# IITD-COMPUTER-VISION-GROUP/Egomotion_with_Local_Loop_Closures

Hardware: AMD Instinct MI355X
Metric: GN iterations/sec (640x480 semi-dense) (higher is better)
Workload: dtype f32; 1 GPU; C2 (configs[2]: batch of 32 loop-closure candidate alignments): 32 different keyframes (own depth map each) against ONE current frame per batch, the reference's loop-closure shape, 640x480, 4-level pyramid, FCA Gauss-Newton, schedule [4, 7, 9, 12] (early exit off), per-call mask compaction included, arithmetic mode 'fast' (pose <= 1e-5 vs the CPU path, tests/test_gpu_fast.py), 16 batches in flight; batch_per_gpu=32, global_batch=32, batches_in_flight=16, coalesce=4, launcher=single process, pixels=semi-dense (maxAbsGradient>=5), arith=fast, cpu_affinity=none

## Files before the change

egomotion_with_local_loop_closures_amd/_lib.py:

```python
import ctypes as C
import os
import subprocess

_HERE = os.path.dirname(os.path.abspath(__file__))
CSRC = os.path.join(_HERE, "csrc")
SO_PATH = os.path.join(CSRC, "libellc_hip.so")
MAX_LEVELS = 8

ABI_SYMBOLS = [
    "ellc_abi_version", "ellc_device_count", "ellc_default_config", "ellc_ctx_create", "ellc_ctx_destroy", "ellc_last_error", "ellc_sync", "ellc_stream", "ellc_ctx_counters", "ellc_ctx_set_poll_timeout_us", "ellc_ctx_set_grid_batch", "ellc_ctx_set_dense_maps", "ellc_ctx_set_persistent_schedule",
    "ellc_frame_upload", "ellc_keyframe_upload", "ellc_keyframe_from_frame", "ellc_get_image_level", "ellc_get_gradient",
    "ellc_get_max_gradient", "ellc_keyframe_set_depth", "ellc_keyframe_set_depth_level", "ellc_keyframe_get_depth_level",
    "ellc_keyframe_set_weights", "ellc_keyframe_get_weights", "ellc_keyframe_finalise_weights", "ellc_align", "ellc_align_enqueue",
    "ellc_align_fetch", "ellc_align_quality_at", "ellc_gn_iterate", "ellc_gn_display_planes", "ellc_concatenate_relative_pose", "ellc_concatenate_origin_pose", "ellc_se3_exp",
    "ellc_se3_log", "ellc_depth_set_state", "ellc_depth_get_state", "ellc_depth_set_keyframe", "ellc_depth_propagate",
    "ellc_depth_observe", "ellc_depth_fill_holes", "ellc_depth_regularize", "ellc_depth_make_inv_depth_one", "ellc_depth_regularize_fill_regularize", "ellc_depth_do_regularization",
    "ellc_depth_update_depth_image", "ellc_depth_create_keyframe", "ellc_depth_seeds", "ellc_track_frame",
    "ellc_histogram", "ellc_kl_divergence", "ellc_copy_slot", "ellc_copy_slot_across",
    "ellc_ingest_configure", "ellc_frame_ingest_bgr",
    "ellc_shard_range", "ellc_comm_unique_id", "ellc_comm_init_rccl", "ellc_comm_init_tcp", "ellc_comm_info", "ellc_comm_destroy", "ellc_comm_last_error",
    "ellc_gather_start", "ellc_gather_finish", "ellc_gather_results",
]


DIAG_SYMBOLS = [
    "ellc_profile_gn_kernel", "ellc_profile_align", "ellc_profile_depth_stage", "ellc_profile_calibrate_read", "ellc_profile_stream_read",
    "ellc_selftest_div_pair", "ellc_selftest_lu", "ellc_debug_persist_delay", "ellc_debug_set_persist_epoch", "ellc_debug_persist_counters", "ellc_debug_set_eager_lists", "ellc_debug_set_hinv_cache", "ellc_debug_set_fold_staging",
    "ellc_debug_set_count_cache", "ellc_debug_count_cache_counters",
    "ellc_debug_schedule_sums",
]


class EllcConfig(C.Structure):
    _fields_ = [("width", C.c_int), ("height", C.c_int), ("levels", C.c_int),
                ("fx", C.c_float), ("fy", C.c_float), ("cx", C.c_float), ("cy", C.c_float),
                ("max_iter", C.c_int * MAX_LEVELS), ("early_exit", C.c_int),
                ("max_keyframes", C.c_int), ("max_frames", C.c_int), ("max_batch", C.c_int), ("device", C.c_int),
                ("concurrent_batches", C.c_int), ("arith", C.c_int), ("coalesce", C.c_int), ("cache_records", C.c_int), ("grid_batch", C.c_int)]


class EllcHypotheses(C.Structure):
    _fields_ = [("invDepth", C.c_void_p), ("invDepthSmoothed", C.c_void_p), ("variance", C.c_void_p), ("varianceSmoothed", C.c_void_p),
                ("validity_counter", C.c_void_p), ("blacklisted", C.c_void_p), ("isValid", C.c_void_p)]


class EllcAlignQuality(C.Structure):
    _fields_ = [("n_depth", C.c_int32), ("n_used", C.c_int32),
                ("sum_r2", C.c_double), ("sum_abs_r", C.c_double), ("sum_w", C.c_double), ("sum_wr2", C.c_double),
                ("H", C.c_float * 36), ("b", C.c_float * 6), ("Hinv", C.c_float * 36)]


class EllcError(RuntimeError):
    pass


def build(verbose=False):
    args = ["make", "-C", CSRC]
    if not verbose:
        args.insert(1, "-s")
    subprocess.check_call(args)

# ... 67 lines not shown
```

egomotion_with_local_loop_closures_amd/api.py:

```python
import ctypes as C
import numpy as np
from . import _lib
from ._lib import EllcConfig, EllcHypotheses, EllcAlignQuality, EllcError, MAX_LEVELS

MODE_FCA = 0
MODE_ICA = 1
ARITH_EXACT = 0
ARITH_FAST = 1
HYP_FIELDS = ("invDepth", "invDepthSmoothed", "variance", "varianceSmoothed", "validity", "blacklisted", "valid")


def _p(a):
    return None if a is None else a.ctypes.data_as(C.c_void_p)


def default_config(width, height, levels=4, **kw):
    cfg = EllcConfig()
    _lib.lib().ellc_default_config(C.byref(cfg), width, height, levels)
    for k, v in kw.items():
        if k == "max_iter":
            mi = list(v) + [12] * (MAX_LEVELS - len(v))
            for i in range(MAX_LEVELS):
                cfg.max_iter[i] = mi[i]
        else:
# ... 271 lines not shown
        self._ck(self._l.ellc_histogram(self.h, int(is_kf), slot, _p(h)), "ellc_histogram")
        return h

    def copy_slot(self, dst_is_kf, dst, src_is_kf, src):
        self._ck(self._l.ellc_copy_slot(self.h, int(dst_is_kf), dst, int(src_is_kf), src), "ellc_copy_slot")

    def _need_diag(self, what):
        if not self.diag and _lib.DIAG_SO_PATH != _lib.SO_PATH:
            raise EllcError("%s is a diagnostic entry point (include/ellc_abi_diag.h): create the context with diag=True" % what)

    def debug_persist_delay(self, first_block, polls):
        self._need_diag("ellc_debug_persist_delay")
        self._ck(self._l.ellc_debug_persist_delay(self.h, int(first_block), int(polls)), "ellc_debug_persist_delay")

    def debug_set_persist_epoch(self, epoch):
        self._need_diag("ellc_debug_set_persist_epoch")
        self._ck(self._l.ellc_debug_set_persist_epoch(self.h, C.c_uint(epoch)), "ellc_debug_set_persist_epoch")

    def debug_set_eager_lists(self, on):
        self._need_diag("ellc_debug_set_eager_lists")
        self._ck(self._l.ellc_debug_set_eager_lists(self.h, int(bool(on))), "ellc_debug_set_eager_lists")

    def debug_set_fold_staging(self, on):
        self._need_diag("ellc_debug_set_fold_staging")
        self._ck(self._l.ellc_debug_set_fold_staging(self.h, int(bool(on))), "ellc_debug_set_fold_staging")

    def debug_set_hinv_cache(self, on):
        self._need_diag("ellc_debug_set_hinv_cache")
        self._ck(self._l.ellc_debug_set_hinv_cache(self.h, int(bool(on))), "ellc_debug_set_hinv_cache")

    def debug_set_count_cache(self, on):
        self._need_diag("ellc_debug_set_count_cache")
        self._ck(self._l.ellc_debug_set_count_cache(self.h, int(bool(on))), "ellc_debug_set_count_cache")

    def debug_count_cache_counters(self):
        self._need_diag("ellc_debug_count_cache_counters")
        a = C.c_longlong(0); b = C.c_longlong(0)
        self._ck(self._l.ellc_debug_count_cache_counters(self.h, C.byref(a), C.byref(b)), "ellc_debug_count_cache_counters")
        return a.value, b.value

    def debug_persist_counters(self):
        self._need_diag("ellc_debug_persist_counters")
        a = C.c_longlong(0); b = C.c_longlong(0); r = C.c_longlong(0)
        self._ck(self._l.ellc_debug_persist_counters(self.h, C.byref(a), C.byref(b), C.byref(r)), "ellc_debug_persist_counters")
        return a.value, b.value, r.value

    def debug_schedule_sums(self, kf_slots, frame_slots, level, pose, mode=MODE_FCA):
        self._need_diag("ellc_debug_schedule_sums")
        B = len(kf_slots)
        pose = np.ascontiguousarray(np.broadcast_to(np.asarray(pose, np.float32).reshape(-1, 6), (B, 6)), np.float32)
        _, kf, fr, _ = self._batch(kf_slots, frame_slots, None)
        sums = np.zeros((B, 27), np.float64); newp = np.zeros((B, 6), np.float32); hinv = np.zeros((B, 36), np.float32)
        name = C.create_string_buffer(64); grid = np.zeros(3, np.int32)
        self._ck(self._l.ellc_debug_schedule_sums(self.h, B, _p(kf), _p(fr), level, mode, _p(pose), _p(sums), _p(newp), _p(hinv), name, 64,
                                                  _p(grid)), "ellc_debug_schedule_sums")
        H = np.zeros((B, 6, 6), np.float64)
        iu = np.triu_indices(6)
        H[:, iu[0], iu[1]] = sums[:, :21]
        H[:, iu[1], iu[0]] = sums[:, :21]
        return dict(H=H, b=sums[:, 21:].copy(), pose=newp, hinv=hinv.reshape(B, 6, 6), kernel=name.value.decode(),
                    grid=tuple(int(v) for v in grid))

    def profile_gn_kernel(self, kf_slots, frame_slots, level, reps=20):
        self._need_diag("ellc_profile_gn_kernel")
        B, kf, fr, _ = self._batch(kf_slots, frame_slots, None)
        ms = C.c_float(0); by = C.c_double(0); v = C.c_longlong(0)
# ... 85 lines not shown
```

egomotion_with_local_loop_closures_amd/csrc/ellc_context.hpp:

```cpp
#pragma once
#include <hip/hip_runtime.h>
#include <string>
#include <vector>
#include <array>
#include <map>
#include <tuple>
#include "../../include/ellc_abi.h"
#ifdef ELLC_DIAG_ABI
#include "../../include/ellc_abi_diag.h"
#endif
#include "ellc_device.hpp"

namespace ellc {

struct DepthSoA {
  float* invDepth = nullptr;
  float* invDepthSmoothed = nullptr;
  float* variance = nullptr;
  float* varianceSmoothed = nullptr;
  int* validity = nullptr;
  int* blacklisted = nullptr;
  uint8_t* isValid = nullptr;
};

struct LaunchPlan {
  int B = 0;
  int nu = 0;
  int mode = ELLC_MODE_FCA;
  int save_weights = 0;
  int set = 0;
  bool continuation = false;
  bool dense = false;
  int need = 0;
  bool skip_count = false;
  bool pollable = false;
  bool resident = false;
  int adaptive_first = 0;
  bool direct = false;
  bool track = false;
  const void* count_valid = nullptr;
  int count_n = 0;
};

struct TrackRequest {
  const void* count_valid;
  int count_n;
};

struct GraphKey {
  int B, nu, mode, save_weights, continuation, track, pollable, adaptive_first, grid_batch, dense, need, skip_count, set;
  bool operator<(const GraphKey& o) const {
    auto t = [](const GraphKey& k) {
      return std::tie(k.B, k.nu, k.mode, k.save_weights, k.continuation, k.track, k.pollable, k.adaptive_first, k.grid_batch, k.dense, k.need, k.skip_count, k.set);
    };
    return t(*this) < t(o);
  }
};
inline GraphKey graph_key(const LaunchPlan& p, int grid_batch) {
  return GraphKey{p.B, p.nu, p.mode, p.save_weights ? 1 : 0, p.continuation, p.track, p.pollable, p.adaptive_first, grid_batch, p.dense, p.need, p.skip_count, p.set};
}

}

struct ellc_ctx {
  ellc_config cfg;
  hipStream_t stream = nullptr;
  std::string err;
  int L = 0;
  ellc::LevelGeom geom_h[ELLC_MAX_LEVELS];
  ellc::LevelGeom* geom_d = nullptr;
  std::vector<void*> allocs;
  char* arena_base = nullptr;
  size_t arena_size = 0, arena_used = 0;
  bool fast = false;
  std::vector<void*> host_allocs;
  std::vector<ellc::KfLevelDev> kf_tab_h;
  std::vector<ellc::FrLevelDev> fr_tab_h;
  ellc::KfLevelDev* kf_tab_d = nullptr;
  ellc::FrLevelDev* fr_tab_d = nullptr;
  std::vector<char> kf_has_image, kf_has_depth, fr_has_image;
  std::vector<char> kf_dense;
  bool dense_maps_off = false;
#ifdef ELLC_NO_DENSE_QUADS
  bool dense_quads = false;
#else
  bool dense_quads = true;
#endif
  std::vector<int> kf_rec_tag;
  std::vector<char> kf_rec_eager;
  bool eager_lists = true;
  bool fold_staging = true;
  std::vector<char> kf_hinv_ok;
  bool hinv_cache = true;
  std::vector<char> kf_counts_ok;
  bool count_cache = true;
  long long groups_counted = 0, groups_count_skipped = 0;
  bool cache_records = false;
  std::vector<std::array<int, ELLC_MAX_LEVELS>> kf_num_weights;
  std::vector<float*> kf_maxgrad, fr_maxgrad;
  std::vector<int*> kf_maxgrad_count, fr_maxgrad_count;
  std::vector<char> kf_maxgrad_valid, fr_maxgrad_valid;
  int *kf_slot_d = nullptr, *fr_slot_d = nullptr, *uniq_slot_d = nullptr;
  int *kf_slot_h = nullptr, *fr_slot_h = nullptr, *uniq_slot_h = nullptr;
  float *init_pose_d = nullptr, *init_pose_h = nullptr;
  ellc::AlignState *state_d = nullptr, *state_h = nullptr;
  ellc::AlignResult* result_h = nullptr;
  ellc::AlignResult* result_dev_alias = nullptr;
// ... 118 lines not shown
  int track_counts = 0;
  int* track_dev_alias = nullptr;
  float Kinv[9], Kmat[9];
};

namespace ellc {
ellc_status fail(ellc_ctx* c, ellc_status s, const std::string& msg);
ellc_status enqueue_eager_lists(ellc_ctx* c, int slot);
void invalidate_records(ellc_ctx* c, int slot);
void invalidate_lists(ellc_ctx* c, int slot);
#define ELLC_HIP(ctx, expr)                                                                               \
  do {                                                                                                    \
    hipError_t e__ = (expr);                                                                              \
    if (e__ != hipSuccess) return ellc::fail(ctx, ELLC_ERR_HIP, std::string(#expr) + ": " + hipGetErrorString(e__)); \
  } while (0)

ellc_status enter(ellc_ctx* c, bool join);
#define ELLC_ENTER_IMPL(ctx, join)                      \
  do {                                                  \
    if (ctx) {                                          \
      const ellc_status s__ = ellc::enter(ctx, join);   \
      if (s__ != ELLC_OK) return s__;                   \
    }                                                   \
  } while (0)
#define ELLC_ENTER(ctx) ELLC_ENTER_IMPL(ctx, true)
#define ELLC_ENTER_BATCH(ctx) ELLC_ENTER_IMPL(ctx, false)

int choose_nblk(const ellc_ctx* c, int level, int B, bool dense);
ellc_status run_prep(ellc_ctx* c, const LaunchPlan& p);
ellc_status build_depth_pyramid(ellc_ctx* c, int slot);
ellc_status build_depth_pyramid_from(ellc_ctx* c, int slot, int first_level);
ellc_status build_maxgrad(ellc_ctx* c, bool is_kf, int slot);
ellc_status build_image_pyramid(ellc_ctx* c, uint8_t* const* img, hipStream_t st);
ellc_status mark_frame_use(ellc_ctx* c, int slot);
}
```

egomotion_with_local_loop_closures_amd/csrc/ellc_device.hpp:

```cpp
#pragma once
#include <hip/hip_runtime.h>
#include <stdint.h>

#define ELLC_MAX_LEVELS 8
#define ELLC_PART_STRIDE 32
#define ELLC_NBLK_MAX 256
#define ELLC_GN_THREADS 256

namespace ellc {

struct LevelGeom {
  int cols, rows, sw, sh;
  int n;
  float fx, fy, cx, cy;
  float rfx, rfy;
  int divc_ok;
  const double* colA;
  const float* colB;
  const double* rowA;
  const float* rowB;
};

struct __attribute__((packed, aligned(4))) FcaRec {
  uint32_t xyI;
// ... 5 lines not shown
  uint32_t xyI;
  float var, d;
};

struct __attribute__((aligned(16))) IcaRec {
  float X, Y, Z, Ikf;
  float W, sd0, sd1, sd2;
  float sd3, sd4, sd5, pad;
};

struct KfLevelDev {
  uint8_t* img;
  float* depth;
  float* var;
  float* weight;
  uint32_t* cxy;
  float* cZ;
  float* cI;
  FcaRec* crec;
  IcaRec* irec;
  float* hpart;
  float* hinv;
  float* cW;
  float* wlast;
  float* sd;
  int* count;
  int* tile_count;
  float* idepth;
  double* invz;
};

struct FrLevelDev {
  uint8_t* img;
};

#define DM_OBS_REGIONS 64

struct AlignState {
  float pose[6];
  float S[12];
  float delta[6];
  float weighted;
  int level_done;
  int pending;
  int cur_level;
  int it_in_level;
  int iters[ELLC_MAX_LEVELS];
  float H[36];
  float b[6];
  float Hinv[36];
};

struct AlignResult {
  float pose[6];
  float weighted;
  int iters[ELLC_MAX_LEVELS];
  int pad;
};

}
```

egomotion_with_local_loop_closures_amd/csrc/ellc_hip.hip:

```cpp
#include "ellc_context.hpp"
#include "ellc_kernels_image.hpp"
#include "ellc_kernels_gn.hpp"
#include "ellc_kernels_prep.hpp"
#include <cstring>
#include <cmath>
#include <algorithm>
#include <cstdlib>
#include <map>
#include <chrono>
#include <thread>
#include <atomic>
#include <mutex>

using namespace ellc;

static ellc_status resolve_batch(ellc_ctx* c, int set);
static ellc_status launch_group(ellc_ctx* c, int set);

namespace ellc {

ellc_status fail(ellc_ctx* c, ellc_status s, const std::string& msg) {
  if (c) c->err = msg;
  return s;
}
// ... 88 lines not shown
  const bool share = c->cfg.concurrent_batches > 1 && (double)n / (256.0 * per_full) < 100.0;
  const int per = std::max(1, per_full / (share ? 2 : 1));
  int nblk = std::min(ELLC_NBLK_MAX, std::min(by_px, per));
  const int cus = std::max(1, c->resident_blocks / blocks_per_cu);
  if (nblk * B > cus) {
    const int one_per_cu = std::max(1, cus / B);
    if (0.3 * n / (256.0 * one_per_cu) <= 4.0) nblk = std::min(nblk, one_per_cu);
  }
  if (B <= 2 && c->use_fused && c->use_adaptive && c->cfg.early_exit && c->cfg.grid_batch == 0) nblk = std::min(nblk, 128);
  return nblk;
}

static dim3 grid2d(int w, int h, dim3 blk) { return dim3((w + blk.x - 1) / blk.x, (h + blk.y - 1) / blk.y); }

ellc_status build_image_pyramid(ellc_ctx* c, uint8_t* const* img, hipStream_t st) {
  const LevelGeom* g = c->geom_h;
  for (int l = 0; l + 1 < c->L; l += 3) {
    PyrChainArgs a;
    a.steps = std::min(3, c->L - 1 - l);
    a.src = img[l];
    for (int k = 0; k < 4; k++) {
      const int q = std::min(l + k, c->L - 1);
      a.w[k] = g[q].sw;
      a.h[k] = g[q].sh;
    }
    for (int k = 0; k < 3; k++) a.dst[k] = img[std::min(l + 1 + k, c->L - 1)];
    const int dw = g[l + a.steps].sw, dh = g[l + a.steps].sh;
    hipLaunchKernelGGL(pyr_down_chain_u8, dim3((dw + ELLC_PT - 1) / ELLC_PT, (dh + ELLC_PT - 1) / ELLC_PT), dim3(256), 0, st, a);
  }
  ELLC_HIP(c, hipGetLastError());
  return ELLC_OK;
}

static ellc_status upload_pyramid(ellc_ctx* c, uint8_t* const* img, const uint8_t* host, int frame_slot = -1) {
  const LevelGeom* g = c->geom_h;
  hipStream_t st = c->stream;
  if (frame_slot >= 0) {
    if (!c->upload_stream) {
      ELLC_HIP(c, hipStreamCreateWithFlags(&c->upload_stream, hipStreamNonBlocking));
      c->fr_use_ev.assign(c->cfg.max_frames, nullptr);
      c->fr_ready_ev.assign(c->cfg.max_frames, nullptr);
      hipEvent_t all = nullptr;
      ELLC_HIP(c, hipEventCreateWithFlags(&all, hipEventDisableTiming));
      hipError_t e = hipEventRecord(all, c->stream);
      if (e == hipSuccess) e = hipStreamWaitEvent(c->upload_stream, all, 0);
      (void)hipEventDestroy(all);
      ELLC_HIP(c, e);
    }
    st = c->upload_stream;
    if (c->fr_use_ev[frame_slot]) ELLC_HIP(c, hipStreamWaitEvent(st, c->fr_use_ev[frame_slot], 0));
    for (int p = 0; p < ellc_ctx::SETS; p++)
      if (c->batch_set[p].launched) ELLC_HIP(c, hipStreamWaitEvent(st, c->batch_set[p].done, 0));
  }
  const size_t bytes = (size_t)g[0].sw * g[0].sh;
  const int k = c->upload_cursor;
  c->upload_cursor = (c->upload_cursor + 1) % ellc_ctx::UPLOAD_RING;
  if (!c->upload_stage[k]) {
    ELLC_HIP(c, hipHostMalloc((void**)&c->upload_stage[k], bytes, hipHostMallocDefault));
    ELLC_HIP(c, hipEventCreateWithFlags(&c->upload_done[k], hipEventDisableTiming));
  } else {
    ELLC_HIP(c, hipEventSynchronize(c->upload_done[k]));
  }
  std::memcpy(c->upload_stage[k], host, bytes);
  {
    void* stage_dev = nullptr;
    ELLC_HIP(c, hipHostGetDevicePointer(&stage_dev, c->upload_stage[k], 0));
    const int blocks = (int)std::min<size_t>(1024, ((bytes >> 4) + 255) / 256 + 1);
    hipLaunchKernelGGL(ingest_copy_u8, dim3(blocks), dim3(256), 0, st, img[0], (const uint8_t*)stage_dev, bytes);
  }
  const ellc_status s = build_image_pyramid(c, img, st);
  ELLC_HIP(c, hipEventRecord(c->upload_done[k], st));
  if (s != ELLC_OK || frame_slot < 0) return s;
  if (!c->fr_ready_ev[frame_slot]) ELLC_HIP(c, hipEventCreateWithFlags(&c->fr_ready_ev[frame_slot], hipEventDisableTiming));
  ELLC_HIP(c, hipEventRecord(c->fr_ready_ev[frame_slot], st));
  ELLC_HIP(c, hipStreamWaitEvent(c->stream, c->fr_ready_ev[frame_slot], 0));
  return ELLC_OK;
}

ellc_status mark_frame_use(ellc_ctx* c, int slot) {
  if (!c->upload_stream) return ELLC_OK;
  if (!c->fr_use_ev[slot]) ELLC_HIP(c, hipEventCreateWithFlags(&c->fr_use_ev[slot], hipEventDisableTiming));
  ELLC_HIP(c, hipEventRecord(c->fr_use_ev[slot], c->stream));
  return ELLC_OK;
}

ellc_status build_maxgrad(ellc_ctx* c, bool is_kf, int slot) {
  const LevelGeom& g = c->geom_h[0];
  const uint8_t* img = is_kf ? c->kf_tab_h[slot].img : c->fr_tab_h[slot].img;
  float* out = is_kf ? c->kf_maxgrad[slot] : c->fr_maxgrad[slot];
  int* cnt = is_kf ? c->kf_maxgrad_count[slot] : c->fr_maxgrad_count[slot];
  ELLC_HIP(c, hipMemsetAsync(cnt, 0, sizeof(int), c->stream));
  hipLaunchKernelGGL(maxgrad_fused, dim3((g.cols + 31) / 32, (g.rows + 7) / 8), dim3(256), 0, c->stream, img, g.sw, g.cols, g.rows, out, cnt);
  ELLC_HIP(c, hipGetLastError());
  (is_kf ? c->kf_maxgrad_valid : c->fr_maxgrad_valid)[slot] = 1;
  return ELLC_OK;
}

ellc_status build_depth_pyramid(ellc_ctx* c, int slot) { return build_depth_pyramid_from(c, slot, 1); }

ellc_status build_depth_pyramid_from(ellc_ctx* c, int slot, int first_level) {
  for (int l = std::max(1, first_level); l < c->L; l++) {
    const KfLevelDev& s = c->kf_tab_h[(l - 1) * c->cfg.max_keyframes + slot];
    const KfLevelDev& d = c->kf_tab_h[l * c->cfg.max_keyframes + slot];
// ... 48 lines not shown
  ELLC_HIP(c, hipGetLastError());
  return ELLC_OK;
}

ellc_status run_prep(ellc_ctx* c, const LaunchPlan& p) { return run_prep_levels(c, p, 0, c->L - 1, c->stream); }

static void enqueue_ica_hinv(ellc_ctx* c, int n_unique) {
  const PrepArgs a = prep_args(c, 4, 0);
  hipLaunchKernelGGL(ica_hinv, dim3(c->L, n_unique), dim3(ELLC_SOLVE_THREADS), 0, c->stream, a);
}

static bool slot_ok(int s, int n) { return s >= 0 && s < n; }

static int grid_batch(const ellc_ctx* c, int B) {
  if (c->cfg.grid_batch > 0) return c->cfg.grid_batch;
  return (c->coalesce > 1 && B % c->cfg.max_batch == 0) ? c->cfg.max_batch * c->coalesce : B;
}

static GnArgs make_gn_args(ellc_ctx* c, const LaunchPlan& p, int level, int save_w, float* planes) {
  GnArgs a;
  a.geom = c->geom_d;
  a.kf_tab = c->kf_tab_d;
  a.fr_tab = c->fr_tab_d;
  a.kf_slot = c->kf_slot_d;
  a.fr_slot = c->fr_slot_d;
  a.state = c->state_d;
  a.partials = c->partials_d;
  a.planes = planes;
  a.level = level;
  a.max_kf = c->cfg.max_keyframes;
  a.max_fr = c->cfg.max_frames;
  a.nblk = choose_nblk(c, level, grid_batch(c, p.B), p.dense);
  a.save_w = save_w;
  return a;
}

static void launch_fca(ellc_ctx* c, dim3 grd, dim3 blk, const GnArgs& a) {
  if (c->fast) hipLaunchKernelGGL((gn_fca_accumulate<false, false, true>), grd, blk, 0, c->stream, a);
  else if (c->geom_h[0].divc_ok) hipLaunchKernelGGL((gn_fca_accumulate<false, true>), grd, blk, 0, c->stream, a);
  else hipLaunchKernelGGL((gn_fca_accumulate<false, false>), grd, blk, 0, c->stream, a);
}

#if defined(__x86_64__)
__attribute__((target("fma")))
#endif
static bool verify_div_const_fma(float b) {
  const float rb = (float)(1.0 / (double)b);
  for (uint32_t m = 0; m < (1u << 23); m++) {
    uint32_t bits = 0x3f800000u | m;
    float a;
    std::memcpy(&a, &bits, 4);
    const float q = a * rb;
    const float e = __builtin_fmaf(-b, q, a);
    const float r = __builtin_fmaf(e, rb, q);
    if (r != a / b) return false;
  }
  return true;
}
static bool verify_div_const(float b) {
  static std::map<uint32_t, bool> cache;
  static std::mutex cache_mutex;
  std::lock_guard<std::mutex> lock(cache_mutex);
  if (!(b > 0.0f) || !std::isfinite(b)) return false;
#if defined(__x86_64__)
  if (!__builtin_cpu_supports("fma")) return false;
#elif !defined(__FP_FAST_FMAF)
// ... 504 lines not shown
        copy_blocking(c, dRB, rowB.data(), g.rows * 4, hipMemcpyHostToDevice) != hipSuccess) {
      *out = c;
      return fail(c, ELLC_ERR_HIP, "cannot upload the Jacobian tables");
    }
    g.colA = dA; g.rowA = dR; g.colB = dB; g.rowB = dRB;
    c->cap[l] = g.n;
    c->tile_begin[l + 1] = c->tile_begin[l] + (g.n + ELLC_TILE - 1) / ELLC_TILE;
    sw = (sw + 1) / 2;
    sh = (sh + 1) / 2;
  }
  TRY(dev_alloc(c, &c->geom_d, ELLC_MAX_LEVELS));
  if (copy_blocking(c, c->geom_d, c->geom_h, sizeof(LevelGeom) * c->L, hipMemcpyHostToDevice) != hipSuccess) {
    *out = c;
    return fail(c, ELLC_ERR_HIP, "cannot upload the level geometry");
  }
  const int MK = cfg->max_keyframes, MF = cfg->max_frames;
  c->kf_tab_h.assign((size_t)c->L * MK, KfLevelDev());
  c->fr_tab_h.assign((size_t)c->L * MF, FrLevelDev());
  for (int l = 0; l < c->L; l++) {
    const LevelGeom& g = c->geom_h[l];
    const size_t n = g.n, ni = (size_t)g.sw * g.sh;
    const int tiles = c->tile_begin[l + 1] - c->tile_begin[l];
    for (int s = 0; s < MK; s++) {
      KfLevelDev& k = c->kf_tab_h[(size_t)l * MK + s];
      TRY(dev_alloc(c, &k.img, ni + 16));
      TRY(dev_alloc(c, &k.depth, n)); TRY(dev_alloc(c, &k.var, n)); TRY(dev_alloc(c, &k.weight, n));
      TRY(dev_alloc(c, &k.cxy, n)); TRY(dev_alloc(c, &k.cZ, n)); TRY(dev_alloc(c, &k.cI, n));
      TRY(dev_alloc(c, &k.crec, n)); TRY(dev_alloc(c, &k.cW, n)); TRY(dev_alloc(c, &k.wlast, n)); TRY(dev_alloc(c, &k.sd, 6 * n));
      TRY(dev_alloc(c, &k.count, 4)); TRY(dev_alloc(c, &k.tile_count, tiles + 1)); TRY(dev_alloc(c, &k.idepth, n));
      k.invz = nullptr;
      if (!c->fast) TRY(dev_alloc(c, &k.invz, n));
      TRY(dev_alloc(c, &k.irec, n)); TRY(dev_alloc(c, &k.hpart, (size_t)(tiles + 1) * ELLC_PART_STRIDE)); TRY(dev_alloc(c, &k.hinv, 36));
    }
    for (int s = 0; s < MF; s++) TRY(dev_alloc(c, &c->fr_tab_h[(size_t)l * MF + s].img, ni + (size_t)g.sw + 32));
  }
  TRY(dev_alloc(c, &c->kf_tab_d, c->kf_tab_h.size()));
  TRY(dev_alloc(c, &c->fr_tab_d, c->fr_tab_h.size()));
  if (copy_blocking(c, c->kf_tab_d, c->kf_tab_h.data(), c->kf_tab_h.size() * sizeof(KfLevelDev), hipMemcpyHostToDevice) != hipSuccess ||
      copy_blocking(c, c->fr_tab_d, c->fr_tab_h.data(), c->fr_tab_h.size() * sizeof(FrLevelDev), hipMemcpyHostToDevice) != hipSuccess) {
    *out = c;
    return fail(c, ELLC_ERR_HIP, "cannot upload the slot tables");
  }
  c->kf_has_image.assign(MK, 0); c->kf_has_depth.assign(MK, 0); c->fr_has_image.assign(MF, 0);
  c->kf_dense.assign(MK, 0);
  c->kf_num_weights.assign(MK, std::array<int, ELLC_MAX_LEVELS>{});
  c->kf_rec_tag.assign(MK, 0);
  c->kf_rec_eager.assign(MK, 0);
  c->kf_hinv_ok.assign(MK, 0);
  c->kf_counts_ok.assign(MK, 0);
  c->cache_records = cfg->cache_records != 0;
  c->kf_maxgrad.assign(MK, nullptr); c->fr_maxgrad.assign(MF, nullptr);
  c->kf_maxgrad_count.assign(MK, nullptr); c->fr_maxgrad_count.assign(MF, nullptr);
  c->kf_maxgrad_valid.assign(MK, 0); c->fr_maxgrad_valid.assign(MF, 0);
  const size_t n0 = (size_t)cfg->width * cfg->height;
  for (int s = 0; s < MK; s++) { TRY(dev_alloc(c, &c->kf_maxgrad[s], n0)); TRY(dev_alloc(c, &c->kf_maxgrad_count[s], 4)); }
  for (int s = 0; s < MF; s++) { TRY(dev_alloc(c, &c->fr_maxgrad[s], n0)); TRY(dev_alloc(c, &c->fr_maxgrad_count[s], 4)); }
  const int MB = cfg->max_batch;
  c->coalesce = std::max(1, cfg->coalesce);
  c->group_cap = c->coalesce * MB;
  c->max_inflight = c->coalesce > 1 ? (ellc_ctx::STREAMS + 1) * c->coalesce : ellc_ctx::STREAMS;
  c->n_sets = c->max_inflight + 1;
  c->batch_stream[0] = c->stream;
  const size_t CAP = (size_t)c->group_cap;
  for (int p = 0; p < c->n_sets; p++) {
    ellc_ctx::BatchSet& bs = c->batch_set[p];
    TRY(dev_alloc(c, &bs.stage_d, 9 * CAP));
    TRY(host_alloc(c, &bs.stage_h, 9 * CAP));
// ... 182 lines not shown
}
ellc_status ellc_debug_set_persist_epoch(ellc_ctx* c, unsigned epoch) {
  if (!c) return ELLC_ERR_BAD_ARG;
  ELLC_ENTER(c);
  c->persist_epoch = epoch;
  return ELLC_OK;
}
ellc_status ellc_debug_set_eager_lists(ellc_ctx* c, int on) {
  if (!c) return ELLC_ERR_BAD_ARG;
  ELLC_ENTER(c);
  c->eager_lists = on != 0;
  if (!on) std::fill(c->kf_rec_eager.begin(), c->kf_rec_eager.end(), 0);
  return ELLC_OK;
}
ellc_status ellc_debug_set_fold_staging(ellc_ctx* c, int on) {
  if (!c) return ELLC_ERR_BAD_ARG;
  ELLC_ENTER(c);
  c->fold_staging = on != 0;
  c->ride_saved_weights = on != 0;
  return ELLC_OK;
}
ellc_status ellc_debug_set_hinv_cache(ellc_ctx* c, int on) {
  if (!c) return ELLC_ERR_BAD_ARG;
  ELLC_ENTER(c);
  c->hinv_cache = on != 0;
  return ELLC_OK;
}
ellc_status ellc_debug_set_count_cache(ellc_ctx* c, int on) {
  if (!c) return ELLC_ERR_BAD_ARG;
  ELLC_ENTER(c);
  c->count_cache = on != 0;
  return ELLC_OK;
}
ellc_status ellc_debug_count_cache_counters(ellc_ctx* c, long long* groups_counted, long long* groups_skipped) {
  if (!c) return ELLC_ERR_BAD_ARG;
  ELLC_ENTER(c);
  if (groups_counted) *groups_counted = c->groups_counted;
  if (groups_skipped) *groups_skipped = c->groups_count_skipped;
  return ELLC_OK;
}
ellc_status ellc_debug_persist_counters(ellc_ctx* c, long long* resident_launches, long long* abandoned_launches, long long* rejoined_blocks) {
  if (!c) return ELLC_ERR_BAD_ARG;
  ELLC_ENTER(c);
  if (resident_launches) *resident_launches = c->persist_launches;
  if (abandoned_launches) *abandoned_launches = c->persist_abandoned;
  if (rejoined_blocks) {
    unsigned long long v = 0;
    ELLC_HIP(c, hipDeviceSynchronize());
    ELLC_HIP(c, hipMemcpyFromSymbol(&v, HIP_SYMBOL(ellc::g_persist_adoptions), sizeof(v)));
    *rejoined_blocks = (long long)v;
  }
  return ELLC_OK;
}
#endif

ellc_status ellc_ctx_set_dense_maps(ellc_ctx* c, int mode) {
  ELLC_ENTER_BATCH(c);
  if (!c || mode < 0 || mode > 1) return fail(c, ELLC_ERR_BAD_ARG, "ellc_ctx_set_dense_maps: mode 0 (automatic) or 1 (always the lists)");
  if (c->open_set >= 0) {
    const ellc_status s = launch_group(c, c->open_set);
    if (s != ELLC_OK) return s;
  }
  c->dense_maps_off = mode == 1;
  return ELLC_OK;
}

ellc_status ellc_ctx_set_grid_batch(ellc_ctx* c, int n) {
  ELLC_ENTER_BATCH(c);
  if (!c || n < 0 || n > 65536) return fail(c, ELLC_ERR_BAD_ARG, "bad argument");
  if (c->open_set >= 0) {
    const ellc_status s = launch_group(c, c->open_set);
    if (s != ELLC_OK) return s;
  }
  c->cfg.grid_batch = n;
  return ELLC_OK;
}

ellc_status ellc_frame_upload(ellc_ctx* c, int slot, const uint8_t* image) {
  ELLC_ENTER(c);
  if (!c || !image || !slot_ok(slot, c->cfg.max_frames)) return fail(c, ELLC_ERR_BAD_ARG, "ellc_frame_upload: bad argument");
  uint8_t* img[ELLC_MAX_LEVELS];
  for (int l = 0; l < c->L; l++) img[l] = c->fr_tab_h[(size_t)l * c->cfg.max_frames + slot].img;
  const bool own_stream = c->cfg.concurrent_batches <= 1 && c->coalesce <= 1;
  ellc_status s = upload_pyramid(c, img, image, own_stream ? slot : -1);
  if (s != ELLC_OK) return s;
  c->fr_has_image[slot] = 1;
  c->fr_maxgrad_valid[slot] = 0;
  return ELLC_OK;
}

ellc_status ellc_keyframe_upload(ellc_ctx* c, int slot, const uint8_t* image) {
  ELLC_ENTER(c);
  if (!c || !image || !slot_ok(slot, c->cfg.max_keyframes)) return fail(c, ELLC_ERR_BAD_ARG, "ellc_keyframe_upload: bad argument");
  uint8_t* img[ELLC_MAX_LEVELS];
  for (int l = 0; l < c->L; l++) img[l] = c->kf_tab_h[(size_t)l * c->cfg.max_keyframes + slot].img;
  invalidate_records(c, slot);
  ellc_status s = upload_pyramid(c, img, image);
  if (s != ELLC_OK) return s;
  c->kf_has_image[slot] = 1;
  c->kf_dense[slot] = 0;
  c->kf_has_depth[slot] = 0;
  for (int l = 0; l < c->L; l++) {
    ELLC_HIP(c, hipMemsetAsync(c->kf_tab_h[(size_t)l * c->cfg.max_keyframes + slot].weight, 0, (size_t)c->geom_h[l].n * 4, c->stream));
    c->kf_num_weights[slot][l] = 0;
  }
  return build_maxgrad(c, true, slot);
}

ellc_status ellc_keyframe_from_frame(ellc_ctx* c, int kf_slot, int frame_slot) {
  ELLC_ENTER(c);
  if (!c || !slot_ok(kf_slot, c->cfg.max_keyframes) || !slot_ok(frame_slot, c->cfg.max_frames)) return fail(c, ELLC_ERR_BAD_ARG, "bad slot");
  if (!c->fr_has_image[frame_slot]) return fail(c, ELLC_ERR_NOT_READY, "frame slot empty");
  invalidate_records(c, kf_slot);
  for (int l = 0; l < c->L; l++) {
    const LevelGeom& g = c->geom_h[l];
    ELLC_HIP(c, hipMemcpyAsync(c->kf_tab_h[(size_t)l * c->cfg.max_keyframes + kf_slot].img, c->fr_tab_h[(size_t)l * c->cfg.max_frames + frame_slot].img,
                               (size_t)g.sw * g.sh, hipMemcpyDeviceToDevice, c->stream));
// ... 187 lines not shown
      KfLevelDev& d = dc->kf_tab_h[(size_t)l * MK + dst];
      if (src_is_kf) {
        const KfLevelDev& k = sc->kf_tab_h[(size_t)l * SK + src];
        ELLC_HIP(c, hipMemcpyAsync(d.depth, k.depth, (size_t)g.n * 4, hipMemcpyDeviceToDevice, dc->stream));
        ELLC_HIP(c, hipMemcpyAsync(d.var, k.var, (size_t)g.n * 4, hipMemcpyDeviceToDevice, dc->stream));
        if (sc->kf_dense[src]) ELLC_HIP(c, hipMemcpyAsync(d.idepth, k.idepth, (size_t)g.n * 4, hipMemcpyDeviceToDevice, dc->stream));
        if (sc->kf_dense[src] && d.invz) {
          if (k.invz) ELLC_HIP(c, hipMemcpyAsync(d.invz, k.invz, (size_t)g.n * 8, hipMemcpyDeviceToDevice, dc->stream));
          else hipLaunchKernelGGL(invz_plane, dim3((g.n + 255) / 256), dim3(256), 0, dc->stream, d.depth, d.invz, g.n);
        }
        ELLC_HIP(c, hipMemcpyAsync(d.weight, k.weight, (size_t)g.n * 4, hipMemcpyDeviceToDevice, dc->stream));
        dc->kf_num_weights[dst][l] = sc->kf_num_weights[src][l];
      } else {
        ELLC_HIP(c, hipMemsetAsync(d.weight, 0, (size_t)g.n * 4, dc->stream));
        dc->kf_num_weights[dst][l] = 0;
      }
    }
  }
  if (dst_is_kf) {
    dc->kf_has_image[dst] = 1;
    dc->kf_has_depth[dst] = src_is_kf ? sc->kf_has_depth[src] : 0;
    dc->kf_dense[dst] = src_is_kf ? sc->kf_dense[src] : 0;
    if (src_is_kf && sc->kf_maxgrad_valid[src]) {
      const size_t n0 = (size_t)dc->cfg.width * dc->cfg.height;
      ELLC_HIP(c, hipMemcpyAsync(dc->kf_maxgrad[dst], sc->kf_maxgrad[src], n0 * 4, hipMemcpyDeviceToDevice, dc->stream));
      ELLC_HIP(c, hipMemcpyAsync(dc->kf_maxgrad_count[dst], sc->kf_maxgrad_count[src], 4, hipMemcpyDeviceToDevice, dc->stream));
      dc->kf_maxgrad_valid[dst] = 1;
    } else {
      return build_maxgrad(dc, true, dst);
    }
  } else {
    dc->fr_has_image[dst] = 1;
    dc->fr_maxgrad_valid[dst] = 0;
  }
  return ELLC_OK;
}
static ellc_status mark_copy_uses(ellc_ctx* dc, int dst_is_kf, int dst, ellc_ctx* sc, int src_is_kf, int src) {
  ellc_status s = ELLC_OK;
  if (!src_is_kf) s = mark_frame_use(sc, src);
  if (s == ELLC_OK && !dst_is_kf && dc == sc) s = mark_frame_use(dc, dst);
  return s;
}

ellc_status ellc_copy_slot(ellc_ctx* c, int dst_is_kf, int dst, int src_is_kf, int src) {
  ELLC_ENTER(c);
  if (!c || !slot_ok(dst, dst_is_kf ? c->cfg.max_keyframes : c->cfg.max_frames) || !slot_ok(src, src_is_kf ? c->cfg.max_keyframes : c->cfg.max_frames))
    return fail(c, ELLC_ERR_BAD_ARG, "bad slot");
  if (!(src_is_kf ? c->kf_has_image[src] : c->fr_has_image[src])) return fail(c, ELLC_ERR_NOT_READY, "source slot empty");
  if (dst_is_kf == src_is_kf && dst == src) return ELLC_OK;
  const ellc_status st = copy_slot_planes(c, dst_is_kf, dst, c, src_is_kf, src);
  return st != ELLC_OK ? st : mark_copy_uses(c, dst_is_kf, dst, c, src_is_kf, src);
}

ellc_status ellc_copy_slot_across(ellc_ctx* dc, int dst_is_kf, int dst, ellc_ctx* sc, int src_is_kf, int src) {
  if (!dc || !sc) return ELLC_ERR_BAD_ARG;
  if (dc == sc) return ellc_copy_slot(dc, dst_is_kf, dst, src_is_kf, src);
  if (dc->cfg.device != sc->cfg.device || dc->cfg.width != sc->cfg.width || dc->cfg.height != sc->cfg.height || dc->L != sc->L)
    return fail(dc, ELLC_ERR_BAD_ARG, "ellc_copy_slot_across: the contexts differ in device or geometry");
  if (!slot_ok(dst, dst_is_kf ? dc->cfg.max_keyframes : dc->cfg.max_frames) || !slot_ok(src, src_is_kf ? sc->cfg.max_keyframes : sc->cfg.max_frames))
    return fail(dc, ELLC_ERR_BAD_ARG, "bad slot");
  if (!(src_is_kf ? sc->kf_has_image[src] : sc->fr_has_image[src])) return fail(dc, ELLC_ERR_NOT_READY, "source slot empty");
  {
    ellc_ctx* c = sc;
    ELLC_ENTER(c);
    if (!sc->ev_xfer) ELLC_HIP(c, hipEventCreateWithFlags(&sc->ev_xfer, hipEventDisableTiming));
    ELLC_HIP(c, hipEventRecord(sc->ev_xfer, sc->stream));
// ... 4 lines not shown
  ELLC_HIP(c, hipStreamWaitEvent(dc->stream, sc->ev_xfer, 0));
  const ellc_status st = copy_slot_planes(dc, dst_is_kf, dst, sc, src_is_kf, src);
  ELLC_HIP(c, hipEventRecord(dc->ev_xfer, dc->stream));
  if (hipStreamWaitEvent(sc->stream, dc->ev_xfer, 0) != hipSuccess) return fail(sc, ELLC_ERR_HIP, "ellc_copy_slot_across: cannot order the source stream");
  sc->main_dirty = true;
  return st;
}

static int need_of(const ellc_ctx* c, int mode) {
  return mode == ELLC_MODE_ICA ? (c->use_fused ? (c->fast ? 20 : 4) : 1) : (c->fast ? 8 : 2);
}

static bool runs_dense(const ellc_ctx* c, int mode, int B, int save_weights) {
  return !c->dense_maps_off && c->use_fused && c->pipe && mode == ELLC_MODE_FCA && !save_weights && !schedule_is_adaptive(c, mode, B);
}
static bool group_is_dense(const ellc_ctx* c, int mode, int B, int save_weights, const int* slots, int n) {
  bool dense = runs_dense(c, mode, B, save_weights);
  for (int i = 0; i < n; i++) dense = dense && c->kf_dense[slots[i]];
  return dense;
}

static LaunchPlan make_plan(const ellc_ctx* c, int B, int nu, int mode, int save_weights, int set, bool dense, bool resident) {
  LaunchPlan p;
  p.B = B;
  p.nu = dense ? 0 : nu;
  p.mode = mode;
  p.save_weights = save_weights;
  p.set = set;
  p.dense = dense;
  p.need = need_of(c, mode);
  p.resident = resident;
  p.adaptive_first = schedule_is_adaptive(c, mode, B) ? adaptive_first_launches(c, resident) : 0;
  p.direct = launches_directly(c, mode, B);
  return p;
}

static ellc_status enqueue_align_body(ellc_ctx* c, const LaunchPlan& p) {
  enqueue_stage_in(c, p, p.B);
  ellc_status s = ELLC_OK;
  if (p.nu > 0) {
    s = run_prep(c, p);
    if (s != ELLC_OK) return s;
    if (p.need & 4) enqueue_ica_hinv(c, p.nu);
  }
  s = enqueue_schedule(c, p);
  if (s != ELLC_OK) return s;
  if (!c->use_fused)
    hipLaunchKernelGGL(gn_export_results, dim3((p.B + 63) / 64), dim3(64), 0, c->stream, c->state_d, c->result_dev_alias, p.B);
  return ELLC_OK;
}

static ellc_status launch_align_graph(ellc_ctx* c, const LaunchPlan& p, bool count_twin = false) {
  auto body = [&](const LaunchPlan& q) -> ellc_status { return q.continuation ? enqueue_schedule_adaptive(c, q) : enqueue_align_body(c, q); };
  if (p.direct) return body(p);
  auto capture = [&](const LaunchPlan& q) -> ellc_status {
    hipGraph_t graph = nullptr;
    hipGraphExec_t exec = nullptr;
    ELLC_HIP(c, hipStreamBeginCapture(c->stream, hipStreamCaptureModeThreadLocal));
    const ellc_status s = body(q);
    hipError_t e = hipStreamEndCapture(c->stream, &graph);
    if (s != ELLC_OK || e != hipSuccess) {
      if (graph) (void)hipGraphDestroy(graph);
      if (s != ELLC_OK) return s;
      return fail(c, ELLC_ERR_HIP, std::string("hipStreamEndCapture: ") + hipGetErrorString(e));
    }
    e = hipGraphInstantiate(&exec, graph, nullptr, nullptr, 0);
// ... 331 lines not shown
  if (last) free_set(c, set);
  return out;
}

ellc_status ellc_align(ellc_ctx* c, int B, const int* kf_slots, const int* frame_slots, const float* init_pose, int mode, int save_weights,
                       float* out_pose, int* out_iters, float* out_weighted) {
  ELLC_ENTER(c);
  if (c && c->n_inflight > 0) return fail(c, ELLC_ERR_NOT_READY, "ellc_align: fetch the enqueued batches first");
  ellc_status s = ellc_align_enqueue(c, B, kf_slots, frame_slots, init_pose, mode, save_weights);
  if (s != ELLC_OK) return s;
  return ellc_align_fetch(c, B, out_pose, out_iters, out_weighted);
}

__global__ void gn_set_pose0(AlignState* state, const float* pose) {
  AlignState& st = state[0];
  float p[6], S[12];
  for (int i = 0; i < 6; i++) { p[i] = pose[i]; st.pose[i] = p[i]; }
  exp_se3_f32(p, S);
  for (int i = 0; i < 12; i++) st.S[i] = S[i];
  st.level_done = -1;
}

ellc_status ellc_gn_iterate(ellc_ctx* c, int kf_slot, int frame_slot, int level, int mode, int iter, const float* pose, float* H36, float* b6,
                            float* delta6, float* new_pose6, float* weighted, float* planes) {
  ELLC_ENTER(c);
  if (!c || !pose || level < 0 || level >= c->L) return fail(c, ELLC_ERR_BAD_ARG, "bad argument");
  if (c->n_inflight > 0) return fail(c, ELLC_ERR_NOT_READY, "ellc_gn_iterate: fetch the enqueued batches first");
  int nu = 0;
  select_batch_set(c, 0);
  invalidate_records(c, kf_slot);
  ellc_status s = stage_batch(c, 1, &kf_slot, &frame_slot, pose, &nu);
  if (s != ELLC_OK) return s;
  LaunchPlan plan;
  plan.B = 1;
  plan.nu = nu;
  plan.mode = mode;
  plan.need = mode == ELLC_MODE_ICA ? 1 : (c->fast ? 8 : 2);
  enqueue_stage_in(c, plan, 0);
  s = run_prep(c, plan);
  if (s != ELLC_OK) return s;
  hipLaunchKernelGGL(gn_set_pose0, dim3(1), dim3(1), 0, c->stream, c->state_d, c->init_pose_d);
  const size_t n = (size_t)c->geom_h[level].n;
  if (planes) ELLC_HIP(c, hipMemsetAsync(c->planes_d, 0, 10 * n * 4, c->stream));
  GnArgs a = make_gn_args(c, plan, level, 0, planes ? c->planes_d : nullptr);
  const dim3 grd(a.nblk, 1), blk(ELLC_GN_THREADS);
  if (mode == ELLC_MODE_FCA) {
    if (planes && c->fast) hipLaunchKernelGGL((gn_fca_accumulate<true, false, true>), grd, blk, 0, c->stream, a);
    else if (planes && c->geom_h[0].divc_ok) hipLaunchKernelGGL((gn_fca_accumulate<true, true>), grd, blk, 0, c->stream, a);
    else if (planes) hipLaunchKernelGGL((gn_fca_accumulate<true, false>), grd, blk, 0, c->stream, a);
    else launch_fca(c, grd, blk, a);
    launch_solve(c, level, 1, a.nblk, 0, 0);
  } else {
    if (iter == 0) {
      hipLaunchKernelGGL(gn_ica_precompute, grd, blk, 0, c->stream, a, c->cap[level]);
      launch_solve(c, level, 1, a.nblk, 1, 0);
    }
    if (planes) hipLaunchKernelGGL(gn_ica_iterate<true>, grd, blk, 0, c->stream, a, c->cap[level]);
    else hipLaunchKernelGGL(gn_ica_iterate<false>, grd, blk, 0, c->stream, a, c->cap[level]);
    launch_solve(c, level, 1, a.nblk, 2, 0);
  }
  ELLC_HIP(c, hipGetLastError());
  ELLC_HIP(c, hipMemcpyAsync(c->state_h, c->state_d, sizeof(AlignState), hipMemcpyDeviceToHost, c->stream));
  if (planes) {
    ELLC_HIP(c, hipMemcpyAsync(planes, c->planes_d, 10 * n * 4, hipMemcpyDeviceToHost, c->stream));
  }
  ELLC_HIP(c, hipStreamSynchronize(c->stream));
// ... 35 lines not shown
  if (!c->quality_out_h) {
    const size_t nb0 = (size_t)quality_nblk(c, 0);
    ellc_status s = host_alloc(c, &c->quality_stage_h, (size_t)8 * MB);
    if (s == ELLC_OK) s = dev_alloc(c, &c->quality_partials_d, (size_t)MB * nb0 * ELLC_PART_STRIDE);
    if (s == ELLC_OK) s = dev_alloc(c, &c->quality_counts_d, (size_t)MB * nb0 * 2);
    ellc_align_quality* oh = nullptr;
    if (s == ELLC_OK) s = host_alloc(c, &oh, (size_t)MB);
    if (s != ELLC_OK) return s;
    void *da = nullptr, *ds = nullptr;
    ELLC_HIP(c, hipHostGetDevicePointer(&da, oh, 0));
    ELLC_HIP(c, hipHostGetDevicePointer(&ds, c->quality_stage_h, 0));
    c->quality_out_dev_alias = (ellc_align_quality*)da;
    c->quality_stage_dev_alias = (const int*)ds;
    c->quality_out_h = oh;
  }
  for (int b = 0; b < B; b++) {
    c->quality_stage_h[b] = kf_slots[b];
    c->quality_stage_h[MB + b] = frame_slots[b];
  }
  std::memcpy(c->quality_stage_h + 2 * MB, pose, (size_t)B * 6 * sizeof(float));
  QualityArgs qa;
  qa.geom = c->geom_d;
  qa.kf_tab = c->kf_tab_d;
  qa.fr_tab = c->fr_tab_d;
  qa.stage = c->quality_stage_dev_alias;
  qa.partials = c->quality_partials_d;
  qa.counts = c->quality_counts_d;
  qa.out = (QualityRec*)c->quality_out_dev_alias;
  qa.level = level;
  qa.max_kf = c->cfg.max_keyframes;
  qa.max_fr = c->cfg.max_frames;
  qa.nblk = quality_nblk(c, level);
  qa.max_batch = MB;
  const dim3 grd(qa.nblk, B), blk(ELLC_GN_THREADS);
  if (c->fast) hipLaunchKernelGGL((gn_fca_quality<true, false>), grd, blk, 0, c->stream, qa);
  else if (c->geom_h[0].divc_ok) hipLaunchKernelGGL((gn_fca_quality<false, true>), grd, blk, 0, c->stream, qa);
  else hipLaunchKernelGGL((gn_fca_quality<false, false>), grd, blk, 0, c->stream, qa);
  hipLaunchKernelGGL(gn_quality_finish, dim3(B), dim3(ELLC_SOLVE_THREADS), 0, c->stream, qa);
  ELLC_HIP(c, hipGetLastError());
  ELLC_HIP(c, hipStreamSynchronize(c->stream));
  std::memcpy(out, c->quality_out_h, (size_t)B * sizeof(ellc_align_quality));
  return ELLC_OK;
}

ellc_status ellc_gn_display_planes(ellc_ctx* c, int kf_slot, int frame_slot, int level, const float* pose, uint8_t* templateimg,
                                   uint8_t* tobewarpedimg, float* warpedimg, float* origres) {
  ELLC_ENTER(c);
  if (!c || !pose || level < 0 || level >= c->L) return fail(c, ELLC_ERR_BAD_ARG, "bad argument");
  if (c->n_inflight > 0) return fail(c, ELLC_ERR_NOT_READY, "ellc_gn_display_planes: fetch the enqueued batches first");
  int nu = 0;
  select_batch_set(c, 0);
  ellc_status s = stage_batch(c, 1, &kf_slot, &frame_slot, pose, &nu);
  if (s != ELLC_OK) return s;
  LaunchPlan plan;
  plan.B = 1;
  enqueue_stage_in(c, plan, 0);
  hipLaunchKernelGGL(gn_set_pose0, dim3(1), dim3(1), 0, c->stream, c->state_d, c->init_pose_d);
  const LevelGeom& g = c->geom_h[level];
  const size_t n = (size_t)g.n;
  float* warped_d = c->planes_d;
  float* orig_d = c->planes_d + n;
  uint8_t* tmpl_d = (uint8_t*)(c->planes_d + 2 * n);
  uint8_t* tbw_d = tmpl_d + n;
  GnArgs a = make_gn_args(c, plan, level, 0, nullptr);
  dim3 blk(32, 8);
  hipLaunchKernelGGL(gn_display_planes, grid2d(g.cols, g.rows, blk), blk, 0, c->stream, a, tmpl_d, tbw_d, warped_d, orig_d);
  ELLC_HIP(c, hipGetLastError());
  if (templateimg) ELLC_HIP(c, hipMemcpyAsync(templateimg, tmpl_d, n, hipMemcpyDeviceToHost, c->stream));
  if (tobewarpedimg) ELLC_HIP(c, hipMemcpyAsync(tobewarpedimg, tbw_d, n, hipMemcpyDeviceToHost, c->stream));
  if (warpedimg) ELLC_HIP(c, hipMemcpyAsync(warpedimg, warped_d, n * 4, hipMemcpyDeviceToHost, c->stream));
  if (origres) ELLC_HIP(c, hipMemcpyAsync(origres, orig_d, n * 4, hipMemcpyDeviceToHost, c->stream));
  ELLC_HIP(c, hipStreamSynchronize(c->stream));
  return ELLC_OK;
}

void ellc_concatenate_relative_pose(const float* a, const float* b, float* dest) {
  float o[6];
  concat_relative_f32(a, b, o);
  std::memcpy(dest, o, sizeof(o));
}
void ellc_concatenate_origin_pose(const float* a, const float* b, float* dest) {
  float o[6];
  concat_origin_f32(a, b, o);
  std::memcpy(dest, o, sizeof(o));
}
void ellc_se3_exp(const float* pose6, float* T16) {
  float S[12];
  exp_se3_f32(pose6, S);
  std::memcpy(T16, S, sizeof(S));
  T16[12] = T16[13] = T16[14] = 0.0f;
  T16[15] = 1.0f;
}
void ellc_se3_log(const float* T16, float* pose6) {
  float S[12];
  std::memcpy(S, T16, sizeof(S));
  log_se3_f32(S, pose6);
}

#ifdef ELLC_DIAG_ABI
ellc_status ellc_profile_gn_kernel(ellc_ctx* c, int B, const int* kf_slots, const int* frame_slots, int level, int reps, float* avg_ms,
                                   double* algorithmic_bytes, long long* valid_pixels) {
  ELLC_ENTER(c);
  if (!c || level < 0 || level >= c->L || reps < 1) return fail(c, ELLC_ERR_BAD_ARG, "bad argument");
  if (c->n_inflight > 0) return fail(c, ELLC_ERR_NOT_READY, "ellc_profile_gn_kernel: fetch the enqueued batches first");
  int nu = 0;
  select_batch_set(c, 0);
  if (kf_slots)
    for (int b = 0; b < B; b++) invalidate_records(c, kf_slots[b]);
  ellc_status s = stage_batch(c, B, kf_slots, frame_slots, nullptr, &nu, nullptr, true);
  if (s != ELLC_OK) return s;
  const bool dense = group_is_dense(c, ELLC_MODE_FCA, B, 0, kf_slots, B);
  LaunchPlan plan;
  plan.B = B;
  plan.nu = dense ? 0 : nu;
  plan.dense = dense;
  plan.need = c->fast ? 8 : 2;
  enqueue_stage_in(c, plan, 0);
  if (!dense) {
    s = run_prep(c, plan);
    if (s != ELLC_OK) return s;
  }
  hipLaunchKernelGGL(gn_init_state, dim3((B + 63) / 64), dim3(64), 0, c->stream, c->state_d, c->init_pose_d, B, c->L - 1);
  const GnArgs a = make_gn_args(c, plan, level, 0, nullptr);
  const dim3 grd(a.nblk, B), blk(ELLC_GN_THREADS);
  if (c->use_fused) {
    FusedArgs fa = fused_args(c, plan, false, (B % 8 == 0) ? 1 : 0, false);
    level_bound_level(c, plan, fa, level);
    fa.res = nullptr;
    fa.prev_level = level;
    fa.prev_nblk = a.nblk;
    fa.early_exit = 0;
    auto launch = [&]() {
      launch_level_bound(c, plan, grd, blk, fa, c->stream);
      fa.seq++;
    };
    for (int i = 0; i < 3; i++) launch();
    if (c->use_graph) {
      hipGraph_t graph = nullptr;
      hipGraphExec_t exec = nullptr;
      ELLC_HIP(c, hipStreamBeginCapture(c->stream, hipStreamCaptureModeThreadLocal));
      for (int i = 0; i < reps; i++) launch();
      hipError_t e = hipStreamEndCapture(c->stream, &graph);
      if (e == hipSuccess) e = hipGraphInstantiate(&exec, graph, nullptr, nullptr, 0);
      if (graph) (void)hipGraphDestroy(graph);
      if (e != hipSuccess) return fail(c, ELLC_ERR_HIP, std::string("profile graph capture: ") + hipGetErrorString(e));
// ... 272 lines not shown
```

egomotion_with_local_loop_closures_amd/csrc/ellc_ingest_impl.hpp:

```cpp
#pragma once
#include "ellc_context.hpp"
#include <cmath>
#include <vector>

namespace ellc {

struct IngestMapEntry {
  short ix, iy;
  unsigned short frac;
  unsigned short pad;
};

static inline void ingest_inv3x3(const double* S, double* t) {
  const double d0 = S[0] * (S[4] * S[8] - S[5] * S[7]) - S[1] * (S[3] * S[8] - S[5] * S[6]) + S[2] * (S[3] * S[7] - S[4] * S[6]);
  if (d0 == 0.0) { for (int i = 0; i < 9; i++) t[i] = 0.0; return; }
  const double d = 1. / d0;
  t[0] = (S[4] * S[8] - S[5] * S[7]) * d;
  t[1] = (S[2] * S[7] - S[1] * S[8]) * d;
  t[2] = (S[1] * S[5] - S[2] * S[4]) * d;
  t[3] = (S[5] * S[6] - S[3] * S[8]) * d;
  t[4] = (S[0] * S[8] - S[2] * S[6]) * d;
  t[5] = (S[2] * S[3] - S[0] * S[5]) * d;
  t[6] = (S[3] * S[7] - S[4] * S[6]) * d;
  t[7] = (S[1] * S[6] - S[0] * S[7]) * d;
// ... 135 lines not shown
  if (ie != hipSuccess) {
    if (c->ingest_map) (void)hipFree(c->ingest_map);
    if (c->ingest_bgr) (void)hipFree(c->ingest_bgr);
    c->ingest_map = nullptr;
    c->ingest_bgr = nullptr;
    return fail(c, ELLC_ERR_HIP, std::string("ellc_ingest_configure: ") + hipGetErrorString(ie));
  }
  c->ingest_w = orig_w;
  c->ingest_h = orig_h;
  return ELLC_OK;
}

ellc_status ellc_frame_ingest_bgr(ellc_ctx* c, int slot, const uint8_t* bgr, uint8_t* gray_probe, uint8_t* undistorted_probe) {
  ELLC_ENTER(c);
  using namespace ellc;
  if (!c || !bgr || !slot_ok(slot, c->cfg.max_frames)) return fail(c, ELLC_ERR_BAD_ARG, "ellc_frame_ingest_bgr: bad argument");
  if (!c->ingest_map) return fail(c, ELLC_ERR_NOT_READY, "ellc_frame_ingest_bgr: call ellc_ingest_configure first");
  const int w = c->ingest_w, h = c->ingest_h, ow = c->cfg.width, oh = c->cfg.height;
  ELLC_HIP(c, hipMemcpyAsync(c->ingest_bgr, bgr, (size_t)w * h * 3, hipMemcpyHostToDevice, c->stream));
  uint8_t *gd = nullptr, *ud = nullptr;
  if (gray_probe) ELLC_HIP(c, hipMalloc(&gd, (size_t)ow * oh));
  if (undistorted_probe && hipMalloc(&ud, (size_t)ow * oh * 4) != hipSuccess) {
    if (gd) (void)hipFree(gd);
    return fail(c, ELLC_ERR_HIP, "ellc_frame_ingest_bgr: cannot allocate the probe buffer");
  }
  uint8_t* img[ELLC_MAX_LEVELS];
  for (int l = 0; l < c->L; l++) img[l] = c->fr_tab_h[(size_t)l * c->cfg.max_frames + slot].img;
  const LevelGeom* g = c->geom_h;
  dim3 blk(32, 8);
  hipLaunchKernelGGL(ingest_frame, grid2d(ow, oh, blk), blk, 0, c->stream, c->ingest_bgr, w, h, (const IngestMapEntry*)c->ingest_map, img[0], ow, oh,
                     g[0].sw, gd, ud);
  hipError_t e = hipGetLastError();
  if (e == hipSuccess && build_image_pyramid(c, img, c->stream) != ELLC_OK) e = hipErrorUnknown;
  if (e == hipSuccess && gd) e = hipMemcpyAsync(gray_probe, gd, (size_t)ow * oh, hipMemcpyDeviceToHost, c->stream);
  if (e == hipSuccess && ud) e = hipMemcpyAsync(undistorted_probe, ud, (size_t)ow * oh * 4, hipMemcpyDeviceToHost, c->stream);
  if (e == hipSuccess) e = hipStreamSynchronize(c->stream);
  if (gd) (void)hipFree(gd);
  if (ud) (void)hipFree(ud);
  if (e != hipSuccess) return fail(c, ELLC_ERR_HIP, std::string("ellc_frame_ingest_bgr: ") + hipGetErrorString(e));
  c->fr_has_image[slot] = 1;
  c->fr_maxgrad_valid[slot] = 0;
  return ELLC_OK;
}

}
```

egomotion_with_local_loop_closures_amd/csrc/ellc_kernels_gn.hpp:

```cpp
#pragma once
#include "ellc_device.hpp"
#include "ellc_se3.hpp"

namespace ellc {

#ifdef ELLC_STAMPS
__device__ unsigned long long g_stamps[64];
__device__ unsigned long long g_block_stamps[4 * 8192];
#define ELLC_BSTAMP(slot)                                                                                    \
  do {                                                                                                       \
    if (threadIdx.x == 0) {                                                                                  \
      unsigned long long t__;                                                                                \
      asm volatile("s_memrealtime %0\n\ts_waitcnt lgkmcnt(0)" : "=s"(t__)::"memory");                        \
      const unsigned bid__ = blockIdx.y * gridDim.x + blockIdx.x;                                            \
      if (bid__ < 8192) g_block_stamps[bid__ * 4 + slot] = t__;                                              \
    }                                                                                                        \
  } while (0)
#define ELLC_STAMP(id)                                                                                       \
  do {                                                                                                       \
    if (blockIdx.x == 0 && blockIdx.y == 0 && threadIdx.x == 0) {                                            \
      unsigned long long t__;                                                                                \
      asm volatile("s_memrealtime %0\n\ts_waitcnt lgkmcnt(0)" : "=s"(t__)::"memory");                            \
      g_stamps[id] = t__;                                                                                    \
    }                                                                                                        \
// ... 35 lines not shown
      g_seq_stamps[(off) + ((seq) & 31)] = t__;                                                              \
    }                                                                                                        \
  } while (0)
#else
#define ELLC_SEQSTAMP(off, seq) do { } while (0)
#endif

#define ELLC_GLOBAL __attribute__((address_space(1)))
typedef const ELLC_GLOBAL uint8_t* g_u8;
typedef const ELLC_GLOBAL float* g_f32;
typedef const ELLC_GLOBAL double* g_f64;
typedef const ELLC_GLOBAL uint32_t* g_u32;
template <class T>
__device__ __forceinline__ const ELLC_GLOBAL T* as_global(const T* p) { return (const ELLC_GLOBAL T*)p; }
template <class T>
__device__ __forceinline__ ELLC_GLOBAL T* as_global_rw(T* p) { return (ELLC_GLOBAL T*)p; }

template <int CTRL, int RMASK>
__device__ __forceinline__ float dpp_add(float v) {
  const int x = __builtin_amdgcn_update_dpp(0, __builtin_bit_cast(int, v), CTRL, RMASK, 0xf, false);
  return v + __builtin_bit_cast(float, x);
}
__device__ __forceinline__ float unzero_f(float v) {
  const float C = 0x1.b7cdfep-34f;
  return (v < 0.0f) ? ((v > -C) ? -C : v) : ((v < C) ? C : v);
}

__device__ __forceinline__ int clampi(int v, int lo, int hi) { return v < lo ? lo : (v > hi ? hi : v); }

typedef uint32_t u32_align1 __attribute__((aligned(1)));
__device__ __forceinline__ uint32_t load_u32_unaligned(g_u8 base, unsigned byte_off) {
  return *(const ELLC_GLOBAL u32_align1*)(base + byte_off);
}
template <int N>
__device__ __forceinline__ float byte_f32(uint32_t w) { return (float)((w >> (8 * N)) & 0xffu); }

#define ELLC_LDS __attribute__((address_space(3)))

struct Taps {
  float I;
  float gx, gy;
};

template <bool WANT_GRAD, bool FAST, bool LAT = false>
__device__ __forceinline__ Taps tap_general(g_u8 img, int sw, int cols, int rows, float x1, float y1) {
  Taps o;
  const float fx0 = floorf(x1), fy0 = floorf(y1);
  const float wx = x1 - fx0, wy = y1 - fy0;
  const float omx = 1.0f - wx, omy = 1.0f - wy;
  if (x1 != x1 || y1 != y1) {
    o.I = -1.0f; o.gx = 0.0f; o.gy = 0.0f;
    return o;
  }
  const float nC = (float)(cols - 1), nR = (float)(rows - 1);
  const bool xf_bad = (fx0 < 0.0f) || (fx0 > nC);
  const bool xc_bad = (x1 < 0.0f) || (x1 > nC);
  const bool yf_bad = (fy0 < 0.0f) || (fy0 > nR);
  const bool yc_bad = (y1 < 0.0f) || (y1 > nR);
  const bool v00 = !(xf_bad || yf_bad), v01 = !(xc_bad || yf_bad), v10 = !(xf_bad || yc_bad), v11 = !(xc_bad || yc_bad);
  if (!(v00 || v01 || v10 || v11)) {
    o.I = -1.0f; o.gx = 0.0f; o.gy = 0.0f;
    return o;
  }
  const int x0 = (int)fminf(fmaxf(fx0, -4.0f), nC + 4.0f);
  const int y0 = (int)fminf(fmaxf(fy0, -4.0f), nR + 4.0f);
  const int xb = clampi(x0, 0, cols - 1), xc = clampi(x0 + 1, 0, cols - 1);
// ... 54 lines not shown
    const int xa = clampi(x0 - 1, 0, cols - 1), xd = clampi(x0 + 2, 0, cols - 1);
    const int ya = clampi(y0 - 1, 0, rows - 1), yd = clampi(y0 + 2, 0, rows - 1);
    const unsigned ra = __umul24((unsigned)ya, (unsigned)sw), rd = __umul24((unsigned)yd, (unsigned)sw);
    const float Pba = (float)img[rb + (unsigned)xa], Pbd = (float)img[rb + (unsigned)xd];
    const float Pca = (float)img[rc + (unsigned)xa], Pcd = (float)img[rc + (unsigned)xd];
    const float Pab = (float)img[ra + (unsigned)xb], Pac = (float)img[ra + (unsigned)xc];
    const float Pdb = (float)img[rd + (unsigned)xb], Pdc = (float)img[rd + (unsigned)xc];
    const float sx0 = (x0 <= 0 || x0 >= cols - 1) ? 1.0f : 0.5f;
    const float sx1 = (x0 + 1 <= 0 || x0 + 1 >= cols - 1) ? 1.0f : 0.5f;
    const float sy0 = (y0 <= 0 || y0 >= rows - 1) ? 1.0f : 0.5f;
    const float sy1 = (y0 + 1 <= 0 || y0 + 1 >= rows - 1) ? 1.0f : 0.5f;
    float g00 = sx0 * (Pbc - Pba), g01 = sx1 * (Pbd - Pbb), g10 = sx0 * (Pcc - Pca), g11 = sx1 * (Pcd - Pcb);
    g00 = v00 ? g00 : 0.0f; g01 = v01 ? g01 : 0.0f; g10 = v10 ? g10 : 0.0f; g11 = v11 ? g11 : 0.0f;
    float top = (omx * g00) + (wx * g01);
    float btm = (omx * g10) + (wx * g11);
    o.gx = (omy * top) + (wy * btm);
    float h00 = sy0 * (Pcb - Pab), h01 = sy0 * (Pcc - Pac), h10 = sy1 * (Pdb - Pbb), h11 = sy1 * (Pdc - Pbc);
    h00 = v00 ? h00 : 0.0f; h01 = v01 ? h01 : 0.0f; h10 = v10 ? h10 : 0.0f; h11 = v11 ? h11 : 0.0f;
    top = (omx * h00) + (wx * h01);
    btm = (omx * h10) + (wx * h11);
    o.gy = (omy * top) + (wy * btm);
    if (FAST) { o.gx *= 2.0f; o.gy *= 2.0f; }
  } else {
    o.gx = 0.0f; o.gy = 0.0f;
  }
  return o;
}

struct NoPrefetch { __device__ __forceinline__ void operator()() const {} };
template <class F> struct LatPF { F f; __device__ __forceinline__ void operator()() const { f(); } };
template <class T> struct is_lat_pf { static constexpr bool value = false; };
template <class F> struct is_lat_pf<LatPF<F>> { static constexpr bool value = true; };
template <class F> __device__ __forceinline__ LatPF<F> lat_pf(F f) { return LatPF<F>{f}; }
template <bool WANT_GRAD, bool FAST = false, class AfterIssue = NoPrefetch>
__device__ __forceinline__ Taps tap_point(g_u8 img, int sw, int cols, int rows, float x1, float y1, AfterIssue after_issue = AfterIssue()) {
  Taps o;
  const float fx0 = floorf(x1), fy0 = floorf(y1);
  const float wx = x1 - fx0, wy = y1 - fy0;
  const float omx = 1.0f - wx, omy = 1.0f - wy;
  const bool interior = (__builtin_amdgcn_fmed3f(fx0, 1.0f, (float)(cols - 3)) == fx0) & (__builtin_amdgcn_fmed3f(fy0, 1.0f, (float)(rows - 3)) == fy0);
  if (__builtin_amdgcn_ballot_w64(!interior) == 0ull) {
    const int x0 = (int)fx0, y0 = (int)fy0;
    uint32_t wa = 0, wb, wc, wd = 0;
    const unsigned ob = __umul24((unsigned)y0, (unsigned)sw) + (unsigned)x0 - 1u, oc = ob + (unsigned)sw;
    wb = load_u32_unaligned(img, ob);
    wc = load_u32_unaligned(img, oc);
    if (WANT_GRAD) { wa = load_u32_unaligned(img, ob - (unsigned)sw); wd = load_u32_unaligned(img, oc + (unsigned)sw); }
    __builtin_amdgcn_sched_barrier(0);
    after_issue();
    __builtin_amdgcn_sched_barrier(0);
    const float Pbb = byte_f32<1>(wb), Pbc = byte_f32<2>(wb), Pcb = byte_f32<1>(wc), Pcc = byte_f32<2>(wc);
    if (FAST) {
      const float top = __builtin_fmaf(wx, Pbc - Pbb, Pbb);
      const float btm = __builtin_fmaf(wx, Pcc - Pcb, Pcb);
      o.I = __builtin_fmaf(wy, btm - top, top);
      if (WANT_GRAD) {
        const float Pba = byte_f32<0>(wb), Pbd = byte_f32<3>(wb), Pca = byte_f32<0>(wc), Pcd = byte_f32<3>(wc);
        const float Pab = byte_f32<1>(wa), Pac = byte_f32<2>(wa), Pdb = byte_f32<1>(wd), Pdc = byte_f32<2>(wd);
        const float g00 = Pbc - Pba, g01 = Pbd - Pbb, g10 = Pcc - Pca, g11 = Pcd - Pcb;
        float t2 = __builtin_fmaf(wx, g01 - g00, g00);
        float b2 = __builtin_fmaf(wx, g11 - g10, g10);
        o.gx = __builtin_fmaf(wy, b2 - t2, t2);
        const float h00 = Pcb - Pab, h01 = Pcc - Pac, h10 = Pdb - Pbb, h11 = Pdc - Pbc;
        t2 = __builtin_fmaf(wx, h01 - h00, h00);
        b2 = __builtin_fmaf(wx, h11 - h10, h10);
        o.gy = __builtin_fmaf(wy, b2 - t2, t2);
      } else {
        o.gx = 0.0f; o.gy = 0.0f;
      }
      return o;
    }
    {
      const float top = (omx * Pbb) + (wx * Pbc);
      const float btm = (omx * Pcb) + (wx * Pcc);
      o.I = (omy * top) + (wy * btm);
    }
    if (WANT_GRAD) {
      const float Pba = byte_f32<0>(wb), Pbd = byte_f32<3>(wb), Pca = byte_f32<0>(wc), Pcd = byte_f32<3>(wc);
      const float Pab = byte_f32<1>(wa), Pac = byte_f32<2>(wa), Pdb = byte_f32<1>(wd), Pdc = byte_f32<2>(wd);
      const float g00 = 0.5f * (Pbc - Pba), g01 = 0.5f * (Pbd - Pbb), g10 = 0.5f * (Pcc - Pca), g11 = 0.5f * (Pcd - Pcb);
      float top = (omx * g00) + (wx * g01);
      float btm = (omx * g10) + (wx * g11);
      o.gx = (omy * top) + (wy * btm);
      const float h00 = 0.5f * (Pcb - Pab), h01 = 0.5f * (Pcc - Pac), h10 = 0.5f * (Pdb - Pbb), h11 = 0.5f * (Pdc - Pbc);
      top = (omx * h00) + (wx * h01);
      btm = (omx * h10) + (wx * h11);
      o.gy = (omy * top) + (wy * btm);
    } else {
      o.gx = 0.0f; o.gy = 0.0f;
    }
    return o;
  }
  after_issue();
  return tap_general<WANT_GRAD, FAST, is_lat_pf<AfterIssue>::value>(img, sw, cols, rows, x1, y1);
}

struct TapRows { g_u8 ra, rb, rc, rd; };
__device__ __forceinline__ TapRows tap_rows(g_u8 img, int sw) {
  TapRows r;
  r.rb = img - 1;
  r.ra = r.rb - sw;
  r.rc = r.rb + sw;
  r.rd = r.rc + sw;
  return r;
}
template <int N>
__device__ __forceinline__ float cvt_ubyte(uint32_t w) {
  float f;
  if (N == 0) asm("v_cvt_f32_ubyte0 %0, %1" : "=v"(f) : "v"(w));
  else if (N == 1) asm("v_cvt_f32_ubyte1 %0, %1" : "=v"(f) : "v"(w));
  else if (N == 2) asm("v_cvt_f32_ubyte2 %0, %1" : "=v"(f) : "v"(w));
  else asm("v_cvt_f32_ubyte3 %0, %1" : "=v"(f) : "v"(w));
  return f;
}
__device__ __forceinline__ int cvt_floor_i32(float x) {
  int i;
  asm("v_cvt_flr_i32_f32 %0, %1" : "=v"(i) : "v"(x));
  return i;
}
struct TapReq {
  uint32_t wa, wb, wc, wd;
  bool interior;
};
template <bool WANT_GRAD, class AfterIssue = NoPrefetch>
__device__ __forceinline__ TapReq tap_request_f(const TapRows& tr, int sw, int cols, int rows, float x1, float y1, AfterIssue after_issue = AfterIssue()) {
  TapReq q;
  q.wa = 0; q.wd = 0;
  const int x0 = cvt_floor_i32(x1), y0 = cvt_floor_i32(y1);
  const bool interior = ((unsigned)(x0 - 1) <= (unsigned)(cols - 4)) & ((unsigned)(y0 - 1) <= (unsigned)(rows - 4));
  q.interior = (__builtin_amdgcn_ballot_w64(!interior) == 0ull);
  q.wb = 0; q.wc = 0;
  if (q.interior) {
    const unsigned off = __umul24((unsigned)y0, (unsigned)sw) + (unsigned)x0;
#ifdef ELLC_X_LDSTAPS
    __shared__ uint32_t xl[4 * 1024 + 4];
    const unsigned o = (off >> 2) & 1023u, shb = (off & 3u) * 8u;
    q.wb = __builtin_amdgcn_alignbit(xl[o + 1], xl[o], shb);
    q.wc = __builtin_amdgcn_alignbit(xl[1024 + o + 1], xl[1024 + o], shb);
    if (WANT_GRAD) { q.wa = __builtin_amdgcn_alignbit(xl[2048 + o + 1], xl[2048 + o], shb); q.wd = __builtin_amdgcn_alignbit(xl[3072 + o + 1], xl[3072 + o], shb); }
#else
    q.wb = load_u32_unaligned(tr.rb, off);
    q.wc = load_u32_unaligned(tr.rc, off);
    if (WANT_GRAD) { q.wa = load_u32_unaligned(tr.ra, off); q.wd = load_u32_unaligned(tr.rd, off); }
#endif
    __builtin_amdgcn_sched_barrier(0);
    after_issue();
    __builtin_amdgcn_sched_barrier(0);
  } else {
    after_issue();
  }
  return q;
}
template <bool WANT_GRAD, bool LAT = false>
__device__ __forceinline__ Taps tap_finish_f(const TapReq& q, g_u8 img, int sw, int cols, int rows, float x1, float y1) {
  if (q.interior) {
    Taps o;
    const float wx = __builtin_amdgcn_fractf(x1), wy = __builtin_amdgcn_fractf(y1);
    const float Pbb = cvt_ubyte<1>(q.wb), Pbc = cvt_ubyte<2>(q.wb), Pcb = cvt_ubyte<1>(q.wc), Pcc = cvt_ubyte<2>(q.wc);
    const float top = __builtin_fmaf(wx, Pbc - Pbb, Pbb);
    const float btm = __builtin_fmaf(wx, Pcc - Pcb, Pcb);
    o.I = __builtin_fmaf(wy, btm - top, top);
    if (WANT_GRAD) {
      const float Pba = cvt_ubyte<0>(q.wb), Pbd = cvt_ubyte<3>(q.wb), Pca = cvt_ubyte<0>(q.wc), Pcd = cvt_ubyte<3>(q.wc);
      const float Pab = cvt_ubyte<1>(q.wa), Pac = cvt_ubyte<2>(q.wa), Pdb = cvt_ubyte<1>(q.wd), Pdc = cvt_ubyte<2>(q.wd);
      const float g00 = Pbc - Pba, g01 = Pbd - Pbb, g10 = Pcc - Pca, g11 = Pcd - Pcb;
      float t2 = __builtin_fmaf(wx, g01 - g00, g00);
      float b2 = __builtin_fmaf(wx, g11 - g10, g10);
      o.gx = __builtin_fmaf(wy, b2 - t2, t2);
      const float h00 = Pcb - Pab, h01 = Pcc - Pac, h10 = Pdb - Pbb, h11 = Pdc - Pbc;
      t2 = __builtin_fmaf(wx, h01 - h00, h00);
      b2 = __builtin_fmaf(wx, h11 - h10, h10);
      o.gy = __builtin_fmaf(wy, b2 - t2, t2);
    } else {
      o.gx = 0.0f; o.gy = 0.0f;
    }
    return o;
  }
  return tap_general<WANT_GRAD, true, LAT>(img, sw, cols, rows, x1, y1);
}

__device__ __forceinline__ float div_const(float a, float b, float rb) {
  const float q = a * rb;
  const float e = __builtin_fmaf(-b, q, a);
  return __builtin_fmaf(e, rb, q);
}

__device__ __forceinline__ void div_pair_ieee(float a0, float b0, float a1, float b1, float& q0, float& q1) {
  typedef float v2 __attribute__((ext_vector_type(2)));
  bool vd0, vd1, vn0, vn1;
  const v2 ds = {__builtin_amdgcn_div_scalef(a0, b0, false, &vd0), __builtin_amdgcn_div_scalef(a1, b1, false, &vd1)};
  const v2 ns = {__builtin_amdgcn_div_scalef(a0, b0, true, &vn0), __builtin_amdgcn_div_scalef(a1, b1, true, &vn1)};
  const v2 r = {__builtin_amdgcn_rcpf(ds.x), __builtin_amdgcn_rcpf(ds.y)};
  const v2 nds = -ds;
  const v2 f0 = __builtin_elementwise_fma(nds, r, (v2)(1.0f));
  const v2 f1 = __builtin_elementwise_fma(f0, r, r);
  const v2 mul = ns * f1;
  const v2 f2 = __builtin_elementwise_fma(nds, mul, ns);
// ... 46 lines not shown
  J[0] = jt0 + jb0;
  J[1] = jt1 + jb1;
  J[2] = jt2 + jb2;
  J[3] = jt3 + 0.0f;
  J[4] = 0.0f + jb4;
  J[5] = jt5 + jb5;
}

__device__ __forceinline__ float fca_weight(const Warp& w, float d, float residual, float gradx, float grady, float s,
                                            const LevelGeom& g, float tx, float ty, float tz) {
  const float gx = g.fx * gradx;
  const float gy = g.fy * grady;
  const float den = (w.pz * w.pz) * d;
  float g0, g1;
  div_pair_ieee(tx * w.pz - tz * w.px, den, ty * w.pz - tz * w.py, den, g0, g1);
  const float drpdd = gx * g0 + gy * g1;
  const float w_p = 1.0f / (16.0f + (s * drpdd) * drpdd);
  const float weighted_rp = fabsf(residual * sqrtf(w_p));
  const float wh = fabsf(weighted_rp < 1.5f ? 1.0f : 1.5f / weighted_rp);
  return wh * w_p;
}

struct GnArgs {
  const LevelGeom* geom;
  const KfLevelDev* kf_tab;
  const FrLevelDev* fr_tab;
  const int* kf_slot;
  const int* fr_slot;
  AlignState* state;
  float* partials;
  float* planes;
  int level, max_kf, max_fr, nblk;
  int save_w;
};

template <int NV>
struct WaveRows {
  static constexpr int N1 = (NV + 1) / 2, N2 = (N1 + 1) / 2;
};
template <int NV>
__device__ __forceinline__ void wave_sum_rows(const float (&v)[NV], float (&out)[WaveRows<NV>::N2]) {
  constexpr int N1 = WaveRows<NV>::N1, N2 = WaveRows<NV>::N2;
  float s1[N1];
#pragma unroll
  for (int j = 0; j < N1; j++) {
    const float a = v[2 * j], b = (2 * j + 1 < NV) ? v[2 * j + 1] : 0.0f;
    const auto t = __builtin_amdgcn_permlane32_swap(__builtin_bit_cast(unsigned, a), __builtin_bit_cast(unsigned, b), false, false);
    const unsigned t0 = t[0], t1 = t[1];
    s1[j] = __builtin_bit_cast(float, t0) + __builtin_bit_cast(float, t1);
  }
#pragma unroll
  for (int j = 0; j < N2; j++) {
    const float a = s1[2 * j], b = (2 * j + 1 < N1) ? s1[2 * j + 1] : 0.0f;
    const auto t = __builtin_amdgcn_permlane16_swap(__builtin_bit_cast(unsigned, a), __builtin_bit_cast(unsigned, b), false, false);
    const unsigned t0 = t[0], t1 = t[1];
    out[j] = __builtin_bit_cast(float, t0) + __builtin_bit_cast(float, t1);
  }
#pragma unroll
  for (int j = 0; j < N2; j++) out[j] = dpp_add<0xB1, 0xf>(out[j]);
#pragma unroll
  for (int j = 0; j < N2; j++) out[j] = dpp_add<0x4E, 0xf>(out[j]);
#pragma unroll
  for (int j = 0; j < N2; j++) out[j] = dpp_add<0x141, 0xf>(out[j]);
#pragma unroll
  for (int j = 0; j < N2; j++) out[j] = dpp_add<0x140, 0xf>(out[j]);
}

// ... 98 lines not shown
  const Warp w = warp_point<true>(in.X, in.Y, in.Z, g, S);
  const Taps t = tap_point<true, false, PF>(cur, g.sw, g.cols, g.rows, w.wx, w.wy, pf);
  FcaPix o;
  jacobian_row_pre(t.gx, t.gy, pre, o.J);
  const bool oob = (t.I == -1.0f);
  o.residual = oob ? 0.0f : (t.I - in.Ikf);
  o.wgt = oob ? 0.0f : fca_weight(w, pre.d, o.residual, t.gx, t.gy, 1.0f * in.var, g, S[3], S[7], S[11]);
  if (a.save_w) *(ELLC_GLOBAL float*)((ELLC_GLOBAL char*)K.wlast + i * 4u) = o.wgt;
  if (DEBUG) {
    const int x = (int)(in.xy & 0xffffu), y = (int)(in.xy >> 16);
    const size_t n = (size_t)g.n, p = (size_t)y * g.cols + x;
    a.planes[0 * n + p] = o.residual;
    a.planes[1 * n + p] = o.wgt;
    a.planes[2 * n + p] = oob ? -1.0f : w.wx;
    a.planes[3 * n + p] = oob ? -1.0f : w.wy;
#pragma unroll
    for (int k = 0; k < 6; k++) a.planes[(4 + k) * n + p] = o.J[k];
  }
  return o;
}

template <bool DEBUG, bool DIVC, class PF = NoPrefetch>
__device__ __forceinline__ FcaPix fca_pixel_in(const GnArgs& a, const KfLevelDev& K, const LevelGeom& g, g_u8 cur,
                                               const float* S, unsigned i, const FcaIn& in, PF pf = PF()) {
  return fca_pixel_pre<DEBUG, PF>(a, K, g, cur, S, i, in, fca_prepare<DIVC>(g, in), pf);
}

template <bool DEBUG, bool DIVC>
__device__ __forceinline__ FcaPix fca_pixel(const GnArgs& a, const KfLevelDev& K, const LevelGeom& g, g_u8 cur,
                                            const float* S, unsigned i) {
  return fca_pixel_in<DEBUG, DIVC>(a, K, g, cur, S, i, fca_load<DIVC>(K, g, i));
}

typedef uint32_t u32x4_t __attribute__((ext_vector_type(4)));
struct FcaInF { u32x4_t v; };
__device__ __forceinline__ FcaInF fcaf_empty() { FcaInF in; in.v = (u32x4_t){0u, 0u, 0x3f800000u, 0u}; return in; }

#define ELLC_FREC 12u
typedef uint32_t Rec12 __attribute__((ext_vector_type(3), aligned(4)));
__device__ __forceinline__ FcaInF fcaf_load_off(const KfLevelDev& K, unsigned byte_off) {
  FcaInF in;
  const Rec12 r = *(const ELLC_GLOBAL Rec12*)((const ELLC_GLOBAL char*)K.crec + byte_off);
  const uint32_t a = r.x, b = r.y, c = r.z;
  in.v = (u32x4_t){a, b, c, 0u};
  return in;
}
__device__ __forceinline__ FcaInF fcaf_load(const KfLevelDev& K, unsigned i) { return fcaf_load_off(K, i * ELLC_FREC); }
__device__ __forceinline__ void fcaf_position_at(const KfLevelDev& K, const LevelGeom& g, int i, int& x, int& y) {
  const uint32_t w = *(const ELLC_GLOBAL uint32_t*)((const ELLC_GLOBAL char*)K.crec + (unsigned)i * 12u);
  x = (int)(w & 0xfffu); y = (int)((w >> 12) & 0xfffu);
}

struct FcafConst {
  float P[12];
  float rfy, qc;
  float rfx, pc;
  float hfx, hfy;
};
__device__ __forceinline__ FcafConst fcaf_const(const LevelGeom& g, const float* S) {
  FcafConst c;
#pragma unroll
  for (int k = 0; k < 4; k++) {
    c.P[k] = __builtin_fmaf(g.fx, S[k], g.cx * S[8 + k]);
    c.P[4 + k] = __builtin_fmaf(g.fy, S[4 + k], g.cy * S[8 + k]);
    c.P[8 + k] = S[8 + k];
  }
  c.rfy = g.rfy; c.qc = -(g.cy * g.rfy);
// ... 107 lines not shown
}
template <bool FLIP = false>
__device__ __forceinline__ void fca_acc_unpack(const FcaAcc& A, float (&o)[27]) {
  o[0] = A.h[0].x; o[1] = A.h[0].y; o[2] = A.h[1].x; o[3] = A.h[1].y; o[4] = A.h[2].x; o[5] = A.h[2].y;
  o[6] = A.h[3].y; o[7] = A.h[4].x; o[8] = A.h[4].y; o[9] = A.h[5].x; o[10] = A.h[5].y;
  o[11] = A.h[6].x; o[12] = A.h[6].y; o[13] = A.h[7].x; o[14] = A.h[7].y;
  o[15] = A.h[8].y; o[16] = A.h[9].x; o[17] = A.h[9].y;
  o[18] = A.h[10].x; o[19] = A.h[10].y;
  o[20] = A.h[11].y;
  o[21] = A.b[0].x; o[22] = A.b[0].y; o[23] = A.b[1].x; o[24] = A.b[1].y; o[25] = A.b[2].x; o[26] = A.b[2].y;
  if (FLIP) {
    o[1] = -o[1]; o[2] = -o[2]; o[3] = -o[3]; o[4] = -o[4];
    o[10] = -o[10]; o[14] = -o[14]; o[17] = -o[17]; o[19] = -o[19];
    o[21] = -o[21]; o[26] = -o[26];
  }
}

template <bool DEBUG, bool DIVC, bool FAST = false>
__global__ __launch_bounds__(ELLC_GN_THREADS) void gn_fca_accumulate(GnArgs a) {
  const int b = blockIdx.y;
  const AlignState& st = a.state[b];
  if (st.level_done == a.level) return;
  const LevelGeom g = a.geom[a.level];
  const KfLevelDev K = a.kf_tab[a.level * a.max_kf + a.kf_slot[b]];
  const FrLevelDev& F = a.fr_tab[a.level * a.max_fr + a.fr_slot[b]];
  const int V = *K.count;
  const int chunk = (V + a.nblk - 1) / a.nblk;
  const int begin = blockIdx.x * chunk;
  const int end = min(V, begin + chunk);
  float S[12];
#pragma unroll
  for (int i = 0; i < 12; i++) S[i] = st.S[i];
  g_u8 cur = as_global(F.img);
  FcaAcc acc;
  fca_acc_zero(acc);
  const TapRows tr = tap_rows(cur, g.sw);
  const FcafConst fc = fcaf_const(g, S);
  for (int i = begin + (int)threadIdx.x; i < end; i += ELLC_GN_THREADS) {
    FcaPix p;
    if constexpr (FAST) p = fcaf_pixel<DEBUG>(a, K, g, cur, tr, fc, (unsigned)i, fcaf_load(K, (unsigned)i));
    else p = fca_pixel<DEBUG, DIVC>(a, K, g, cur, S, i);
    fca_accumulate_pixel(acc, p);
  }
  float sums[27];
  fca_acc_unpack<FAST>(acc, sums);
  block_reduce_store<27>(sums, a.partials + ((size_t)b * ELLC_NBLK_MAX + blockIdx.x) * ELLC_PART_STRIDE);
}

__global__ __launch_bounds__(ELLC_GN_THREADS) void gn_ica_precompute(GnArgs a, int cap) {
  const int b = blockIdx.y;
  const AlignState& st = a.state[b];
  if (st.level_done == a.level) return;
  const LevelGeom g = a.geom[a.level];
  const KfLevelDev K = a.kf_tab[a.level * a.max_kf + a.kf_slot[b]];
  const int V = *K.count;
  const int chunk = (V + a.nblk - 1) / a.nblk;
  const int begin = blockIdx.x * chunk;
  const int end = min(V, begin + chunk);
  const int stride = ELLC_GN_THREADS;
  g_u8 img = as_global(K.img);
  float acc[21];
#pragma unroll
  for (int i = 0; i < 21; i++) acc[i] = 0.0f;
  for (int i = begin + (int)threadIdx.x; i < end; i += stride) {
    const uint32_t xy = as_global(K.cxy)[i];
    const int x = (int)(xy & 0xffffu), y = (int)(xy >> 16);
    const float Z = as_global(K.cZ)[i];
    const int xm = clampi(x - 1, 0, g.cols - 1), xp = clampi(x + 1, 0, g.cols - 1);
    const int ym = clampi(y - 1, 0, g.rows - 1), yp = clampi(y + 1, 0, g.rows - 1);
// ... 626 lines not shown
  tc.rem = __builtin_amdgcn_readfirstlane((end - begin) - tc.n_full * ELLC_GN_THREADS);
  tc.n_steps = tc.n_full + (tc.rem > 0 ? 1 : 0);
  return tc;
}

__device__ __forceinline__ void plane_xy(int i, int cols, int& x, int& y) {
  y = (int)(((float)i + 0.5f) * (1.0f / (float)cols));
  if (y * cols > i) y--;
  if ((y + 1) * cols <= i) y++;
  x = i - y * cols;
}
struct PlaneWalk { int cols, qstep, rstep; };
struct PlanePos { int i, x, y; };
__device__ __forceinline__ PlaneWalk plane_walk(int cols) {
  PlaneWalk w;
  w.cols = cols;
  w.qstep = ELLC_GN_THREADS / cols;
  w.rstep = ELLC_GN_THREADS - w.qstep * cols;
  return w;
}
__device__ __forceinline__ PlanePos plane_first(const PlaneWalk& w, const Chunk& c, int t) {
  PlanePos p = {c.begin + t, 0, 0};
  if (c.begin < c.end) plane_xy(min(p.i, c.end - 1), w.cols, p.x, p.y);
  return p;
}
__device__ __forceinline__ PlanePos plane_next(const PlaneWalk& w, const PlanePos& p, int last) {
  PlanePos n = {p.i + ELLC_GN_THREADS, p.x + w.rstep, p.y + w.qstep};
  if (n.x >= w.cols) { n.x -= w.cols; n.y++; }
  if (n.i > last) plane_xy(last, w.cols, n.x, n.y);
  return n;
}

template <bool DIVC, bool PIPE, bool FAST, int SAVEW, bool LAT = false>
__device__ __forceinline__ void fca_chunk_pass(const GnArgs& a, const KfLevelDev& K, const LevelGeom& g, g_u8 cur, const float* newS, int begin,
                                               int end, const FcaIn& first, const FcaInF& firstf, const FcaPre& first_pre, float (&sums)[27]) {
  constexpr int stride = ELLC_GN_THREADS;
  const int t = threadIdx.x;
  float S[12];
#pragma unroll
  for (int i = 0; i < 12; i++) S[i] = newS[i];
  FcaAcc acc;
  fca_acc_zero(acc);
  int i = begin + t;
  if constexpr (FAST) {
    if (begin < end) {
      const TapRows tr = tap_rows(cur, g.sw);
      const FcafConst fc = fcaf_const(g, S);
      ELLC_PTRACE(4, 0);
      unsigned off = (unsigned)i * ELLC_FREC, idx = (unsigned)i;
      const unsigned off_last = (unsigned)(end - 1) * ELLC_FREC;
      constexpr unsigned S16 = stride * ELLC_FREC;
      const TripCount tc = trip_count(begin, end);
      FcaInF r0 = firstf, r1 = firstf;
      auto step = [&](const FcaInF& cur_rec, FcaInF& next_rec, bool active) {
        auto refill = [&]() { next_rec = fcaf_load_off(K, min(off + S16, off_last)); };
        const FcafStage st = fcaf_stage_a(g, tr, fc, cur_rec, refill);
        ELLC_PTRACE(5, 0);
        if (active) fca_accumulate_pixel(acc, fcaf_stage_b<false, SAVEW, LAT>(a, K, g, cur, fc, idx, st));
        ELLC_PTRACE(6, 0);
        off += S16; idx += stride;
      };
      for (int k = 0; k < tc.n_steps; k += 2) {
        step(r0, r1, tc.active(k));
        if (k + 1 >= tc.n_steps) break;
        step(r1, r0, tc.active(k + 1));
      }
    }
  } else if (i < end) {
    if (PIPE) {
      FcaIn r0 = first, r1 = first;
      {
        const int i1 = i + stride;
        auto prefetch = [&]() { r1 = fca_load<DIVC>(K, g, (unsigned)min(i1, end - 1)); };
        if constexpr (LAT) fca_accumulate_pixel(acc, fca_pixel_pre<false>(a, K, g, cur, S, (unsigned)i, first, first_pre, lat_pf(prefetch)));
        else fca_accumulate_pixel(acc, fca_pixel_pre<false>(a, K, g, cur, S, (unsigned)i, first, first_pre, prefetch));
        i += stride;
      }
      auto step = [&](const FcaIn& in, FcaIn& fill) {
        const int i1 = i + stride;
// ... 8 lines not shown
        step(r0, r1);
      }
    } else {
      fca_accumulate_pixel(acc, fca_pixel_pre<false>(a, K, g, cur, S, (unsigned)i, first, first_pre));
      for (i += stride; i < end; i += stride) {
        const FcaPix q = fca_pixel<false, DIVC>(a, K, g, cur, S, (unsigned)i);
        fca_accumulate_pixel(acc, q);
      }
    }
  }
  fca_acc_unpack<FAST>(acc, sums);
}

template <bool DIVC, bool PIPE, bool FAST = false, int SAVEW = -1>
__global__ __launch_bounds__(ELLC_GN_THREADS, 4) void gn_fca_fused(const AlignState* src_state, const float* prev_part, int prev_nblk,
                                                                   int nblk, int age_rounds, FusedArgs fa) {
  const GnArgs& a = fa.g;
  const BlockMap m = block_map(nblk, age_rounds, fa.xcd_map);
  const int b = m.b, sub = m.sub;
  const AlignState& src = src_state[b];
  __shared__ SolveShared sh;
  const int t = threadIdx.x;
  ELLC_STAMP(0);
  ELLC_BSTAMP(0);
  ELLC_SEQSTAMP(0, fa.seq);
  const LevelGeom g = a.geom[a.level];
  const KfLevelDev K = a.kf_tab[a.level * a.max_kf + a.kf_slot[b]];
  const FrLevelDev& F = a.fr_tab[a.level * a.max_fr + a.fr_slot[b]];
  const int pending = src.pending;
  const int V = *as_global(K.count);
  const double group_sum = partial_group_sum(pending_partials(prev_part, b), prev_nblk);
  const Chunk c = m.chunk(fa.age_cum, V, nblk);
  g_u8 cur = as_global(F.img);
  FirstRec first = no_record();
  request_first<DIVC, FAST, true>(first, K, g, c, t, true);
  advance_pose<FAST>(sh, pending, group_sum, 0, fa.prev_level, fa.early_exit, src);
  ELLC_STAMP(6);
  ELLC_BSTAMP(1);
  if (publish_level_bound(sh, src, next_state(fa, b), sub == 0, pending, fa.prev_level, a.level)) return;
  float sums[27];
  fca_chunk_pass<DIVC, PIPE, FAST, SAVEW>(a, K, g, cur, sh.newS, c.begin, c.end, first.in, first.inf, first.pre, sums);
  ELLC_STAMP(7);
  ELLC_BSTAMP(2);
  block_reduce_store<27>(sums, partial_record(fa, fa.seq, b, sub));
  ELLC_STAMP(8);
  ELLC_BSTAMP(3);
  ELLC_SEQSTAMP(32, fa.seq);
}

struct DensePix { float Z, var; uint32_t I; };
__device__ __forceinline__ DensePix dense_request(const KfLevelDev& K, unsigned i, unsigned img_off) {
  DensePix p;
  p.Z = as_global(K.depth)[i];
  p.var = as_global(K.var)[i];
  p.I = (uint32_t)as_global(K.img)[img_off];
  return p;
}
__device__ __forceinline__ FcaInF dense_form(const LevelGeom& g, const DensePix& p, int x, int y, bool& valid) {
  valid = p.Z > 0.0f;
  FcaInF in;
  const float dd = __builtin_amdgcn_rcpf(valid ? p.Z : 1.0f);
  in.v = (u32x4_t){(uint32_t)x | ((uint32_t)y << 12) | (p.I << 24), __builtin_bit_cast(uint32_t, p.var), __builtin_bit_cast(uint32_t, dd), 0u};
  return in;
}
template <class Pix, class Request, class Step>
__device__ __forceinline__ void dense_plane_pass(const Chunk& c, const PlaneWalk& w, int sw, PlanePos p, Pix& pix, Request request, Step step) {
  const TripCount tc = trip_count(c.begin, c.end);
  for (int k = 0; k < tc.n_steps; k++) {
    const PlanePos n = plane_next(w, p, c.end - 1);
    auto refill = [&]() { pix = request((unsigned)min(n.i, c.end - 1), (unsigned)(n.y * sw + n.x)); };
    step(pix, p, tc.active(k), refill);
    p = n;
  }
}

__global__ __launch_bounds__(ELLC_GN_THREADS, 4) void gn_fca_dense(const AlignState* src_state, const float* prev_part, int prev_nblk, int nblk, int age_rounds,
                                                                   FusedArgs fa) {
  const GnArgs& a = fa.g;
  const BlockMap m = block_map(nblk, age_rounds, fa.xcd_map);
  const int b = m.b, sub = m.sub;
  const AlignState& src = src_state[b];
  __shared__ SolveShared sh;
  const int t = threadIdx.x;
  const LevelGeom g = a.geom[a.level];
  const KfLevelDev K = a.kf_tab[a.level * a.max_kf + a.kf_slot[b]];
  const FrLevelDev& F = a.fr_tab[a.level * a.max_fr + a.fr_slot[b]];
  const int pending = src.pending;
  const double group_sum = partial_group_sum(pending_partials(prev_part, b), prev_nblk);
  const Chunk c = m.chunk(fa.age_cum, g.n, nblk);
  g_u8 cur = as_global(F.img);
  const int sw = g.sw;
  const PlaneWalk w = plane_walk(g.cols);
  const PlanePos p0 = plane_first(w, c, t);
  DensePix pix;
  pix.Z = 0.0f; pix.var = 0.0f; pix.I = 0u;
  if (c.begin < c.end) pix = dense_request(K, (unsigned)min(p0.i, c.end - 1), (unsigned)(p0.y * sw + p0.x));
  advance_pose<true>(sh, pending, group_sum, 0, fa.prev_level, fa.early_exit, src);
  if (publish_level_bound(sh, src, next_state(fa, b), sub == 0, pending, fa.prev_level, a.level)) return;
  float sums[27];
  {
    float S[12];
#pragma unroll
    for (int i = 0; i < 12; i++) S[i] = sh.newS[i];
    FcaAcc acc;
    fca_acc_zero(acc);
    if (c.begin < c.end) {
      const TapRows tr = tap_rows(cur, sw);
      const FcafConst fc = fcaf_const(g, S);
      dense_plane_pass(c, w, sw, p0, pix, [&](unsigned i, unsigned img_off) { return dense_request(K, i, img_off); },
                       [&](const DensePix& px, const PlanePos& p, bool active, auto refill) {
                         bool valid;
                         const FcaInF rec = dense_form(g, px, p.x, p.y, valid);
                         const FcafStage st = fcaf_stage_a(g, tr, fc, rec, refill);
                         if (active && valid) fca_accumulate_pixel(acc, fcaf_stage_b<false, 0>(a, K, g, cur, fc, (unsigned)p.i, st));
                       });
    }
    fca_acc_unpack<true>(acc, sums);
  }
  block_reduce_store<27>(sums, partial_record(fa, fa.seq, b, sub));
}

struct DensePixX { float Z, var; uint32_t I; double invZ; };
__device__ __forceinline__ DensePixX dense_request_x(const KfLevelDev& K, unsigned i, unsigned img_off) {
  DensePixX p;
  p.Z = as_global(K.depth)[i];
  p.var = as_global(K.var)[i];
  p.I = (uint32_t)as_global(K.img)[img_off];
  p.invZ = ((const ELLC_GLOBAL double*)K.invz)[i];
  return p;
}
template <bool DIVC>
__global__ __launch_bounds__(ELLC_GN_THREADS, 4) void gn_fca_dense_x(const AlignState* src_state, const float* prev_part, int prev_nblk, int nblk, int age_rounds,
                                                                     FusedArgs fa) {
  const GnArgs& a = fa.g;
  const BlockMap m = block_map(nblk, age_rounds, fa.xcd_map);
  const int b = m.b, sub = m.sub;
  const AlignState& src = src_state[b];
  __shared__ SolveShared sh;
  const int t = threadIdx.x;
  const LevelGeom g = a.geom[a.level];
// ... 10 lines not shown
  pix.Z = 0.0f; pix.var = 0.0f; pix.I = 0u; pix.invZ = 1.0;
  if (c.begin < c.end) pix = dense_request_x(K, (unsigned)min(p0.i, c.end - 1), (unsigned)(p0.y * sw + p0.x));
  advance_pose<false>(sh, pending, group_sum, 0, fa.prev_level, fa.early_exit, src);
  if (publish_level_bound(sh, src, next_state(fa, b), sub == 0, pending, fa.prev_level, a.level)) return;
  float sums[27];
  {
    float S[12];
#pragma unroll
    for (int i = 0; i < 12; i++) S[i] = sh.newS[i];
    FcaAcc acc;
    fca_acc_zero(acc);
    if (c.begin < c.end)
      dense_plane_pass(c, w, sw, p0, pix, [&](unsigned i, unsigned img_off) { return dense_request_x(K, i, img_off); },
                       [&](const DensePixX& px, const PlanePos& p, bool active, auto refill) {
                         const bool valid = px.Z > 0.0f;
                         FcaIn in;
                         in.xy = ((uint32_t)p.y << 16) | (uint32_t)p.x;
                         in.Ikf = (float)px.I;
                         in.Z = valid ? px.Z : 1.0f;
                         in.var = px.var;
                         in.invZ = valid ? px.invZ : 1.0;
                         const float aX = ((float)p.x - g.cx) * in.Z, aY = ((float)p.y - g.cy) * in.Z;
                         in.X = DIVC ? div_const(aX, g.fx, g.rfx) : aX / g.fx;
                         in.Y = DIVC ? div_const(aY, g.fy, g.rfy) : aY / g.fy;
                         const FcaPix q = fca_pixel_in<false, DIVC>(a, K, g, cur, S, (unsigned)p.i, in, refill);
                         if (active && valid) fca_accumulate_pixel(acc, q);
                       });
    fca_acc_unpack<false>(acc, sums);
  }
  block_reduce_store<27>(sums, partial_record(fa, fa.seq, b, sub));
}

typedef float f32x4_t __attribute__((ext_vector_type(4)));
typedef uint32_t u32x2_t __attribute__((ext_vector_type(2)));
typedef u32x2_t u32x2_a1 __attribute__((aligned(1)));
struct QuadPlanes { f32x4_t Z, var; uint32_t I; };
__device__ __forceinline__ QuadPlanes quad_request(const KfLevelDev& K, unsigned i4, unsigned img_off) {
  QuadPlanes p;
  const unsigned boff = i4 << 2;
  p.Z = *(const ELLC_GLOBAL f32x4_t*)((const ELLC_GLOBAL char*)K.idepth + boff);
  p.var = *(const ELLC_GLOBAL f32x4_t*)((const ELLC_GLOBAL char*)K.var + boff);
  p.I = *(const ELLC_GLOBAL uint32_t*)((const ELLC_GLOBAL char*)K.img + img_off);
  return p;
}
#define ELLC_QUAD_BLOCKS_PER_CU 3
#define ELLC_QUAD_QCAP (64 + 4 * 64)
#ifdef ELLC_QUAD_STATS
__device__ unsigned long long g_quad_stats[4];
#endif

__global__ __launch_bounds__(ELLC_GN_THREADS, ELLC_QUAD_BLOCKS_PER_CU) void gn_fca_dense4(const AlignState* src_state, const float* prev_part, int prev_nblk, int nblk, int age_rounds,
                                                                    FusedArgs fa) {
  ELLC_BSTAMP(0);
  const GnArgs& a = fa.g;
  const BlockMap m = block_map(nblk, age_rounds, fa.xcd_map);
  const int b = m.b, sub = m.sub;
  const AlignState& src = src_state[b];
  __shared__ SolveShared sh;
  __shared__ uint32_t qbuf[ELLC_GN_THREADS / 64][ELLC_QUAD_QCAP];
  const int t = threadIdx.x;
  const LevelGeom g = a.geom[a.level];
  const KfLevelDev K = a.kf_tab[a.level * a.max_kf + a.kf_slot[b]];
  const FrLevelDev& F = a.fr_tab[a.level * a.max_fr + a.fr_slot[b]];
  const int pending = src.pending;
  const int cols = g.cols, sw = g.sw;
  const int cols4 = cols >> 2;
  const double group_sum = partial_group_sum(pending_partials(prev_part, b), prev_nblk);
  const Chunk c = m.chunk(fa.age_cum, g.n >> 2, nblk);
  const int begin = c.begin, end = c.end;
  g_u8 cur = as_global(F.img);
  const PlaneWalk w = plane_walk(cols4);
  PlanePos p = plane_first(w, c, t);
  QuadPlanes pl;
  pl.Z = (f32x4_t)(0.0f); pl.var = (f32x4_t)(0.0f); pl.I = 0u;
  if (begin < end)
    pl = quad_request(K, 4u * (unsigned)min(p.i, end - 1), __umul24((unsigned)p.y, (unsigned)sw) + 4u * (unsigned)p.x);
  advance_pose<true>(sh, pending, group_sum, 0, fa.prev_level, fa.early_exit, src);
  ELLC_BSTAMP(1);
  if (publish_level_bound(sh, src, next_state(fa, b), sub == 0, pending, fa.prev_level, a.level)) return;
  float sums[27];
  {
    float S[12];
#pragma unroll
    for (int i = 0; i < 12; i++) S[i] = __builtin_bit_cast(float, __builtin_amdgcn_readfirstlane(__builtin_bit_cast(int, sh.newS[i])));
    FcaAcc acc;
    fca_acc_zero(acc);
    if (begin < end) {
      const TapRows tr = tap_rows(cur, sw);
      const g_u8 row_e = tr.rd + sw;
      float P[12];
      {
        const FcafConst f0 = fcaf_const(g, S);
#pragma unroll
        for (int i = 0; i < 12; i++) P[i] = __builtin_bit_cast(float, __builtin_amdgcn_readfirstlane(__builtin_bit_cast(int, f0.P[i])));
      }
      const float s_rfy = g.rfy, s_qc = -(g.cy * g.rfy), s_pc = -(g.cx * g.rfx);
      float vP0 = P[0], vP3 = P[3], vP4 = P[4], vP7 = P[7], vP8 = P[8], vP11 = P[11], v_rfx = g.rfx, v_hfx = 0.5f * g.fx, v_hfy = 0.5f * g.fy;
      asm volatile("" : "+v"(vP0), "+v"(vP3), "+v"(vP4), "+v"(vP7), "+v"(vP8), "+v"(vP11), "+v"(v_rfx), "+v"(v_hfx), "+v"(v_hfy));
      const TripCount tc = trip_count(begin, end);
      const int lane = t & 63;
      uint32_t* const q = qbuf[t >> 6];
      int qn = 0;
      for (int k = 0;; k++) {
        const bool more = (k < tc.n_steps);
        if (more) {
          const bool active = tc.active(k);
          const f32x4_t cZ = pl.Z, cvar = pl.var;
          const uint32_t cI = pl.I;
          const unsigned i4 = 4u * (unsigned)min(p.i, end - 1);
          const int x = 4 * p.x, yrow = p.y;
          const PlanePos n = plane_next(w, p, end - 1);
          const unsigned inext = 4u * (unsigned)min(n.i, end - 1);
          const bool v0 = cZ.x > 0.0f, v1 = cZ.y > 0.0f, v2 = cZ.z > 0.0f, v3 = cZ.w > 0.0f;
          float d0 = cZ.x, d1 = cZ.y, d2 = cZ.z, d3 = cZ.w;
          if (__builtin_amdgcn_ballot_w64(!(v0 && v1 && v2 && v3)) != 0ull) {
            const float dref = v0 ? d0 : (v1 ? d1 : (v2 ? d2 : (v3 ? d3 : 1.0f)));
            d0 = v0 ? d0 : dref; d1 = v1 ? d1 : dref; d2 = v2 ? d2 : dref; d3 = v3 ? d3 : dref;
          }
          const float dd[4] = {d0, d1, d2, d3};
          const bool vv[4] = {v0, v1, v2, v3};
          const float p0 = __builtin_fmaf((float)x, v_rfx, s_pc), qq = __builtin_fmaf((float)yrow, s_rfy, s_qc);
          const float bqx = __builtin_fmaf(P[1], qq, P[2]), bqy = __builtin_fmaf(P[5], qq, P[6]), bqz = __builtin_fmaf(P[9], qq, P[10]);
          float x1[4], y1[4], hrz[4];
          int x0[4], y0[4];
          int xs, xm, ys, ym;
          {
            float pj = p0;
#pragma unroll
            for (int j = 0; j < 4; j++) {
              const float px = __builtin_fmaf(vP0, pj, __builtin_fmaf(vP3, dd[j], bqx));
              const float py = __builtin_fmaf(vP4, pj, __builtin_fmaf(vP7, dd[j], bqy));
              const float pz = __builtin_fmaf(vP8, pj, __builtin_fmaf(vP11, dd[j], bqz));
              const float rz = __builtin_amdgcn_rcpf(pz);
              x1[j] = px * rz; y1[j] = py * rz; hrz[j] = 0.5f * rz;
              x0[j] = cvt_floor_i32(x1[j]); y0[j] = cvt_floor_i32(y1[j]);
              pj += v_rfx;
            }
            xs = min(min(x0[0], x0[1]), min(x0[2], x0[3])); xm = max(max(x0[0], x0[1]), max(x0[2], x0[3]));
            ys = min(min(y0[0], y0[1]), min(y0[2], y0[3])); ym = max(max(y0[0], y0[1]), max(y0[2], y0[3]));
          }
          const bool fit = ((unsigned)(xs - 1) <= (unsigned)(cols - 4)) & ((unsigned)(xm - 1) <= (unsigned)(cols - 4)) &
                           ((unsigned)(ys - 1) <= (unsigned)(g.rows - 4)) & ((unsigned)(ym - 1) <= (unsigned)(g.rows - 4)) &
                           (xm - xs <= 4) & (ym - ys <= 1);
          const unsigned off = fit ? __umul24((unsigned)ys, (unsigned)sw) + (unsigned)xs : (unsigned)sw + 1u;
          const u32x2_t wA = *(const ELLC_GLOBAL u32x2_a1*)(tr.ra + off);
          const u32x2_t wB = *(const ELLC_GLOBAL u32x2_a1*)(tr.rb + off);
          const u32x2_t wC = *(const ELLC_GLOBAL u32x2_a1*)(tr.rc + off);
          const u32x2_t wD = *(const ELLC_GLOBAL u32x2_a1*)(tr.rd + off);
          const u32x2_t wE = *(const ELLC_GLOBAL u32x2_a1*)(row_e + off);
          __builtin_amdgcn_sched_barrier(0);
          pl = quad_request(K, inext, __umul24((unsigned)n.y, (unsigned)sw) + 4u * (unsigned)n.x);
          __builtin_amdgcn_sched_barrier(0);
          const float var[4] = {cvar.x, cvar.y, cvar.z, cvar.w};
          const uint32_t wAx = wA.x, wAy = wA.y, wBx = wB.x, wBy = wB.y, wCx = wC.x, wCy = wC.y, wDx = wD.x, wDy = wD.y, wEx = wE.x, wEy = wE.y;
          float pj = p0;
#pragma unroll
          for (int j = 0; j < 4; j++) {
            const float fx_ = __builtin_amdgcn_fractf(x1[j]), fy_ = __builtin_amdgcn_fractf(y1[j]);
            const uint32_t s1 = (uint32_t)(x0[j] - xs);
            const uint32_t sel = __builtin_amdgcn_perm(s1, s1, 0u) + 0x03020100u;
            const bool dy = (y0[j] != ys);
            const uint32_t r0 = __builtin_amdgcn_perm(wAy, wAx, sel), r1 = __builtin_amdgcn_perm(wBy, wBx, sel), r2 = __builtin_amdgcn_perm(wCy, wCx, sel);
            const uint32_t r3 = __builtin_amdgcn_perm(wDy, wDx, sel), r4 = __builtin_amdgcn_perm(wEy, wEx, sel);
            const uint32_t qa = dy ? r1 : r0, qb = dy ? r2 : r1, qc = dy ? r3 : r2, qd = dy ? r4 : r3;
            const float Pbb = cvt_ubyte<1>(qb), Pbc = cvt_ubyte<2>(qb), Pcb = cvt_ubyte<1>(qc), Pcc = cvt_ubyte<2>(qc);
            const float top = __builtin_fmaf(fx_, Pbc - Pbb, Pbb);
            const float btm = __builtin_fmaf(fx_, Pcc - Pcb, Pcb);
            const float I = __builtin_fmaf(fy_, btm - top, top);
            const float Pba = cvt_ubyte<0>(qb), Pbd = cvt_ubyte<3>(qb), Pca = cvt_ubyte<0>(qc), Pcd = cvt_ubyte<3>(qc);
            const float Pab = cvt_ubyte<1>(qa), Pac = cvt_ubyte<2>(qa), Pdb = cvt_ubyte<1>(qd), Pdc = cvt_ubyte<2>(qd);
            const float g00 = Pbc - Pba, g01 = Pbd - Pbb, g10 = Pcc - Pca, g11 = Pcd - Pcb;
            float t2 = __builtin_fmaf(fx_, g01 - g00, g00);
            float b2 = __builtin_fmaf(fx_, g11 - g10, g10);
            const float gx = __builtin_fmaf(fy_, b2 - t2, t2);
            const float h00 = Pcb - Pab, h01 = Pcc - Pac, h10 = Pdb - Pbb, h11 = Pdc - Pbc;
            t2 = __builtin_fmaf(fx_, h01 - h00, h00);
            b2 = __builtin_fmaf(fx_, h11 - h10, h10);
            const float gy = __builtin_fmaf(fy_, b2 - t2, t2);
            FcaPix o;
            const float A = v_hfx * gx, B = v_hfy * gy;
            const float T = __builtin_fmaf(A, pj, B * qq);
// ... 87 lines not shown
      if (t == 0) { dst->weighted = src.weighted; dst->level_done = src.level_done; dst->pending = 0;
                    dst->cur_level = (fa.continuation && fa.seq == 0) ? -2 : lvl; dst->it_in_level = 0; }
    }
    return;
  }
  if (sub >= max(fa.nblk_lv[lvl], lvl > 0 ? fa.nblk_lv[lvl - 1] : 0)) return;
  LevelWork L = level_work(fa, m, lvl, slot, frs);
  const double group_sum = partial_group_sum_from(pend, pv, L.nb);
  FirstRec first = no_record();
  request_first<DIVC, FAST, true>(first, L.K, L.g, L.c, t, sub < L.nb);
  advance_pose<FAST>(sh, pending, group_sum, 0, lvl, fa.early_exit, src);
  const LevelStep ls = level_step(sh, fa, pending, lvl, src.it_in_level);
  if (writer) {
    if (t < 6) dst->pose[t] = sh.newpose[t];
    if (t < 12) dst->S[t] = sh.newS[t];
    if (t < ELLC_MAX_LEVELS) dst->iters[t] = src.iters[t] + ((pending && t == lvl) ? 1 : 0);
    if (t == 0) {
      dst->weighted = sh.weighted;
      dst->level_done = sh.level_done;
      dst->pending = ls.nl >= 0 ? 1 : 0;
      dst->cur_level = ls.nl;
      dst->it_in_level = ls.it;
    }
  }
  if (ls.nl < 0) return;
  if (ls.over) {
    L = level_work(fa, m, ls.nl, slot, frs);
    if (sub >= L.nb) return;
    request_first<DIVC, FAST, false>(first, L.K, L.g, L.c, t, true);
  } else if (sub >= L.nb) {
    return;
  }
  g_u8 cur = as_global(L.F->img);
  float sums[27];
  fca_chunk_pass<DIVC, true, FAST, SAVEW>(a, L.K, L.g, cur, sh.newS, L.c.begin, L.c.end, first.in, first.inf, first.pre, sums);
  block_reduce_store<27>(sums, partial_record(fa, fa.seq, b, sub));
}

#define ELLC_PERSIST_BAR_WORDS 64
#define ELLC_PERSIST_STATE_WORD 32
#define ELLC_PERSIST_SPIN_LIMIT (1u << 15)
__device__ __forceinline__ int persist_word_of(int s) { return s + s / 7; }
__device__ __forceinline__ void persist_store_record(float (&acc)[27], unsigned* out, unsigned tag) {
  __shared__ float red[ELLC_GN_THREADS / 64][32];
  const int lane = threadIdx.x & 63, wave = threadIdx.x >> 6;
  float rows[WaveRows<27>::N2];
  wave_sum_rows<27>(acc, rows);
  ELLC_PTRACE(8, 0);
  if ((lane & 15) == 0) {
    const int q = lane >> 4, col = 2 * (q & 1) + (q >> 1);
#pragma unroll
    for (int j = 0; j < WaveRows<27>::N2; j++) red[wave][4 * j + col] = rows[j];
  }
  __syncthreads();
  ELLC_PTRACE(9, 0);
  if (threadIdx.x < 32) {
    const int w = (int)threadIdx.x, sidx = w - (w >> 3);
    const bool tagl = (w & 7) == 7;
    float v = 0.0f;
    if (!tagl && sidx < 27) {
      v = red[0][sidx];
#pragma unroll
      for (int k = 1; k < ELLC_GN_THREADS / 64; k++) v += red[k][sidx];
    }
    __hip_atomic_store(out + w, tagl ? tag : __builtin_bit_cast(unsigned, v), __ATOMIC_RELAXED, __HIP_MEMORY_SCOPE_AGENT);
  }
}
enum { PERSIST_OK = 0, PERSIST_ABANDON = 1, PERSIST_LAPPED = 2 };
// ... 203 lines not shown
#endif
        seq = s_seq;
        __syncthreads();
        if (t == 0) s_flag = 0;
      } else {
        solve_step<FAST>(sh, group_sum, 0, lvl, fa.early_exit, st, writer ? rec : nullptr);
      }
    } else {
      carry_pose(sh, st);
    }
    ELLC_PTRACE(3, 0);
    LevelStep ls = level_step(sh, fa, pending, lvl, it_in);
    if (adopted) { ls.over = true; ls.nl = s_level; ls.it = 0; }
    if (writer && ls.over) persist_publish_state(state_line, (epoch << 8) | (unsigned)seq, sh, seq, ls.nl);
    if (t < 6) st.pose[t] = sh.newpose[t];
    if (t < 12) st.S[t] = sh.newS[t];
    if (t == lvl && pending) st.iters[t] += 1;
    if (t == 0) {
      st.weighted = sh.weighted;
      st.level_done = sh.level_done;
      st.pending = ls.nl >= 0 ? 1 : 0;
      st.cur_level = ls.nl;
      st.it_in_level = ls.it;
    }
    if (ls.nl < 0) break;
    bool work = sub < L.nb;
    if (ls.over) {
      L = level_work(fa, m, ls.nl, slot, frs);
      work = sub < L.nb;
      if (work) request_first<DIVC, FAST, false>(first, L.K, L.g, L.c, t, true);
    }
    if (work) {
      g_u8 cur = as_global(L.F->img);
      float sums[27];
      fca_chunk_pass<DIVC, true, FAST, SAVEW, true>(a, L.K, L.g, cur, sh.newS, L.c.begin, L.c.end, first.in, first.inf, first.pre, sums);
      ELLC_PTRACE(7, 0);
      unsigned* out = (unsigned*)partial_record(fa, seq, b, sub);
      persist_store_record(sums, out, (epoch << 8) | (unsigned)(seq + 1));
      ELLC_PTRACE(10, 0);
    }
    __syncthreads();
  }
  __syncthreads();
  if (writer) {
    if (t == 0) st.pending = 0;
    __syncthreads();
    fused_finish_body<FAST, true>(fa, b, st, rec, sh);
  }
}

struct IcaIn { float X, Y, Z, Ikf, W, sd[6]; };
__device__ __forceinline__ IcaIn ica_load(const IcaRec* irec, unsigned i) {
  typedef float f32x4 __attribute__((ext_vector_type(4)));
  const ELLC_GLOBAL f32x4* r = (const ELLC_GLOBAL f32x4*)((const ELLC_GLOBAL char*)irec + i * (unsigned)sizeof(IcaRec));
  const f32x4 a = r[0], b = r[1], c = r[2];
  IcaIn in;
  in.X = a.x; in.Y = a.y; in.Z = a.z; in.Ikf = a.w;
  in.W = b.x; in.sd[0] = b.y; in.sd[1] = b.z; in.sd[2] = b.w;
  in.sd[3] = c.x; in.sd[4] = c.y; in.sd[5] = c.z;
  return in;
}
struct IcaInF { uint32_t xyI; float d, W; uint32_t gxy; };
__device__ __forceinline__ IcaInF ica_load_fast(const KfLevelDev& K, unsigned i) {
  typedef uint32_t u32x4 __attribute__((ext_vector_type(4)));
  const u32x4 v = *(const ELLC_GLOBAL u32x4*)((const ELLC_GLOBAL char*)K.crec + i * 16u);
  IcaInF in;
  const uint32_t w1 = v.y, w2 = v.z, w3 = v.w;
  in.xyI = v.x; in.d = __builtin_bit_cast(float, w1); in.W = __builtin_bit_cast(float, w2); in.gxy = w3;
  return in;
}
template <bool FAST> struct IcaInOf { typedef IcaIn type; };
template <> struct IcaInOf<true> { typedef IcaInF type; };
template <bool FAST>
__device__ __forceinline__ typename IcaInOf<FAST>::type ica_load_any(const KfLevelDev& K, unsigned i) {
  if constexpr (FAST) return ica_load_fast(K, i);
  else return ica_load(K.irec, i);
}
template <bool FAST>
__device__ __forceinline__ typename IcaInOf<FAST>::type ica_in_empty() {
  typename IcaInOf<FAST>::type in;
  if constexpr (FAST) {
    in.xyI = 0; in.d = 1.0f; in.W = 0.0f; in.gxy = 0u;
  } else {
    in.X = 0.0f; in.Y = 0.0f; in.Z = 1.0f; in.Ikf = 0.0f; in.W = 0.0f;
#pragma unroll
    for (int r = 0; r < 6; r++) in.sd[r] = 0.0f;
  }
  return in;
}

template <bool FAST>
__device__ __forceinline__ void ica_accumulate_pixel(float (&acc)[6], const typename IcaInOf<FAST>::type& in, const LevelGeom& g, g_u8 cur,
                                                     const float* S) {
  if constexpr (FAST) {
    const float p = __builtin_fmaf((float)(in.xyI & 0xfffu), g.rfx, -(g.cx * g.rfx));
    const float q = __builtin_fmaf((float)((in.xyI >> 12) & 0xfffu), g.rfy, -(g.cy * g.rfy));
    const float d = in.d;
    const float px = __builtin_fmaf(S[0], p, __builtin_fmaf(S[1], q, __builtin_fmaf(S[3], d, S[2])));
    const float py = __builtin_fmaf(S[4], p, __builtin_fmaf(S[5], q, __builtin_fmaf(S[7], d, S[6])));
    const float pz = __builtin_fmaf(S[8], p, __builtin_fmaf(S[9], q, __builtin_fmaf(S[11], d, S[10])));
    const float rz = __builtin_amdgcn_rcpf(pz);
    const float wx = __builtin_fmaf(px * rz, g.fx, g.cx);
    const float wy = __builtin_fmaf(py * rz, g.fy, g.cy);
    const Taps t = tap_point<false, true>(cur, g.sw, g.cols, g.rows, wx, wy);
    const bool oob = (t.I == -1.0f);
    const float residual = oob ? 0.0f : (t.I - byte_f32<3>(in.xyI));
    const float rw = residual * in.W;
    const float A = g.fx * ((float)(int)(short)(in.gxy & 0xffffu) * 0.5f), B = g.fy * ((float)((int)in.gxy >> 16) * 0.5f);
    const float T = __builtin_fmaf(A, p, B * q);
    acc[0] = __builtin_fmaf(-__builtin_fmaf(q, T, B), rw, acc[0]);
    acc[1] = __builtin_fmaf(__builtin_fmaf(p, T, A), rw, acc[1]);
    acc[2] = __builtin_fmaf(__builtin_fmaf(B, p, -(A * q)), rw, acc[2]);
    acc[3] = __builtin_fmaf(A * d, rw, acc[3]);
    acc[4] = __builtin_fmaf(B * d, rw, acc[4]);
    acc[5] = __builtin_fmaf(-(d * T), rw, acc[5]);
  } else {
    const Warp w = warp_point<true>(in.X, in.Y, in.Z, g, S);
    const Taps t = tap_point<false, false>(cur, g.sw, g.cols, g.rows, w.wx, w.wy);
    const bool oob = (t.I == -1.0f);
    const float residual = oob ? 0.0f : (t.I - in.Ikf);
    const float rw = residual * in.W;
#pragma unroll
    for (int r = 0; r < 6; r++) acc[r] = __builtin_fmaf(in.sd[r], rw, acc[r]);
  }
}

template <bool FAST>
__global__ __launch_bounds__(ELLC_GN_THREADS) void gn_ica_fused(const AlignState* src_state, const float* prev_part, int prev_nblk, FusedArgs fa) {
  const GnArgs& a = fa.g;
  const BlockMap m = block_map(a.nblk, 0, 0);
  const int b = m.b, sub = m.sub;
  const AlignState& src = src_state[b];
  __shared__ SolveShared sh;
  const int t = threadIdx.x;
  const LevelGeom g = a.geom[a.level];
  const int slot = a.kf_slot[b];
  const KfLevelDev K = a.kf_tab[a.level * a.max_kf + slot];
  const FrLevelDev& F = a.fr_tab[a.level * a.max_fr + a.fr_slot[b]];
  const int pending = src.pending;
  const int V = *as_global(K.count);
  const double group_sum = partial_group_sum(pending_partials(prev_part, b), prev_nblk);
  const Chunk c = m.chunk(fa.age_cum, V, a.nblk);
  const int begin = c.begin, end = c.end;
  g_u8 cur = as_global(F.img);
  typename IcaInOf<FAST>::type first = ica_in_empty<FAST>();
  if (begin + t < end) first = ica_load_any<FAST>(K, (unsigned)(begin + t));
  advance_pose<FAST>(sh, pending, group_sum, 2, fa.prev_level, fa.early_exit, src, &a.kf_tab[fa.prev_level * a.max_kf + slot].hinv);
  if (publish_level_bound(sh, src, next_state(fa, b), sub == 0, pending, fa.prev_level, a.level)) return;
  float S[12];
#pragma unroll
  for (int i = 0; i < 12; i++) S[i] = sh.newS[i];
  float acc[6];
#pragma unroll
  for (int i = 0; i < 6; i++) acc[i] = 0.0f;
  int i = begin + t;
  if (i < end) {
    ica_accumulate_pixel<FAST>(acc, first, g, cur, S);
    for (i += ELLC_GN_THREADS; i < end; i += ELLC_GN_THREADS) ica_accumulate_pixel<FAST>(acc, ica_load_any<FAST>(K, (unsigned)i), g, cur, S);
  }
  block_reduce_store<6>(acc, partial_record(fa, fa.seq, b, sub) + 21);
}

template <bool FAST, bool ADAPT>
__device__ __forceinline__ void fused_finish_body(const FusedArgs& fa, int b, const AlignState& src, AlignState* dst, SolveShared& sh) {
  const GnArgs& a = fa.g;
  const int t = threadIdx.x;
  const int lvl = ADAPT ? src.cur_level : fa.prev_level;
  const int pending = ADAPT ? (src.pending && lvl >= 0) : src.pending;
  const int it_in = ADAPT ? src.it_in_level : 0;
  __shared__ int it_copy[ELLC_MAX_LEVELS];
  if (t < ELLC_MAX_LEVELS) it_copy[t] = src.iters[t];
  if (pending) {
    const float* hinv = fa.ica ? a.kf_tab[lvl * a.max_kf + a.kf_slot[b]].hinv : nullptr;
    solve_step<FAST>(sh, partial_group_sum(pending_partials(fa, fa.seq, b), ADAPT ? fa.nblk_lv[lvl] : fa.prev_nblk), fa.ica ? 2 : 0, lvl, fa.early_exit, src, dst, hinv);
  } else {
    carry_pose(sh, src);
  }
  LevelStep ls = {false, -1, 0};
  if (ADAPT && lvl >= 0) ls = level_step(sh, fa, pending, lvl, it_in);
  const bool ended = ls.nl < 0;
  if (FAST && ended) {
    if (t == 0) {
      float S[12], np[6];
      for (int i = 0; i < 12; i++) S[i] = sh.newS[i];
      log_se3_f32(S, np);
      for (int i = 0; i < 6; i++) sh.newpose[i] = np[i];
    }
    __syncthreads();
  }
  if (t < 6) dst->pose[t] = sh.newpose[t];
  if (t < 12) dst->S[t] = sh.newS[t];
// ... 175 lines not shown
      p = (size_t)((xyI >> 12) & 0xfffu) * cols + (xyI & 0xfffu);
    }
    K.weight[p] = K.weight[p] + K.wlast[i];
  }
}
__global__ void gn_add_saved_weights_all(const KfLevelDev* kf_tab, const int* kf_slot, const LevelGeom* geom, const AlignState* state, int max_kf,
                                         int fast_records) {
  saved_weights_all_body(kf_tab, kf_slot, geom, state, max_kf, fast_records, (int)blockIdx.y, (int)blockIdx.z, (int)blockIdx.x, (int)gridDim.x, (int)threadIdx.x,
                         (int)blockDim.x);
}
struct RideWeights {
  int n = 0, per_level = 0;
  const KfLevelDev* kf_tab = nullptr;
  const int* kf_slot = nullptr;
  const LevelGeom* geom = nullptr;
  const AlignState* state = nullptr;
  int max_kf = 0, fast_records = 0;
};

struct QualityRec {
  int32_t n_depth, n_used;
  double sum_r2, sum_abs_r, sum_w, sum_wr2;
  float H[36], b[6], Hinv[36];
};
struct QualityArgs {
  const LevelGeom* geom;
  const KfLevelDev* kf_tab;
  const FrLevelDev* fr_tab;
  const int* stage;
  float* partials;
  int* counts;
  QualityRec* out;
  int level, max_kf, max_fr, nblk, max_batch;
};

__device__ __forceinline__ bool tap_oob(int cols, int rows, float x1, float y1) {
  if (x1 != x1 || y1 != y1) return true;
  const float fx0 = floorf(x1), fy0 = floorf(y1);
  const float nC = (float)(cols - 1), nR = (float)(rows - 1);
  const bool xf_bad = (fx0 < 0.0f) || (fx0 > nC);
  const bool xc_bad = (x1 < 0.0f) || (x1 > nC);
  const bool yf_bad = (fy0 < 0.0f) || (fy0 > nR);
  const bool yc_bad = (y1 < 0.0f) || (y1 > nR);
  return (xf_bad && xc_bad) || (yf_bad && yc_bad);
}

#define ELLC_QUALITY_QCAP 128
template <bool FAST, bool DIVC>
__global__ __launch_bounds__(ELLC_GN_THREADS, 4) void gn_fca_quality(QualityArgs qa) {
  const int b = blockIdx.y, sub = blockIdx.x, t = threadIdx.x;
  const LevelGeom g = qa.geom[qa.level];
  const KfLevelDev K = qa.kf_tab[qa.level * qa.max_kf + qa.stage[b]];
  const FrLevelDev& F = qa.fr_tab[qa.level * qa.max_fr + qa.stage[qa.max_batch + b]];
  g_u8 cur = as_global(F.img);
  Chunk c;
  {
    const int n = (g.n + qa.nblk - 1) / qa.nblk;
    c.begin = sub * n;
    c.end = min(g.n, c.begin + n);
  }
  const int sw = g.sw, cols = g.cols;
  const PlaneWalk w = plane_walk(cols);
  PlanePos p = plane_first(w, c, t);
  float z = 0.0f;
  if (c.begin < c.end) z = as_global(K.depth)[(unsigned)min(p.i, c.end - 1)];
  __shared__ float Ssh[12];
  __shared__ uint32_t qbuf[ELLC_GN_THREADS / 64][ELLC_QUALITY_QCAP];
  if (t < 64) {
    const float* pose = (const float*)(qa.stage + 2 * qa.max_batch) + 6 * b;
    const int l9 = min(t, 8);
    const int r3 = l9 / 3, k3 = l9 - 3 * r3;
    double Rrk, Vv;
    exp_se3_entry((double)pose[0], (double)pose[1], (double)pose[2], (double)pose[3], (double)pose[4], (double)pose[5], r3, k3, Rrk, Vv);
    const double trow = (Vv + __shfl_down(Vv, 1)) + __shfl_down(Vv, 2);
    if (t < 9) {
      Ssh[r3 * 4 + k3] = (float)Rrk;
      if (k3 == 0) Ssh[r3 * 4 + 3] = (float)trow;
    }
  }
  __syncthreads();
  float S[12];
#pragma unroll
  for (int i = 0; i < 12; i++) S[i] = Ssh[i];
  GnArgs a;
  a.geom = qa.geom; a.kf_tab = qa.kf_tab; a.fr_tab = qa.fr_tab; a.kf_slot = nullptr; a.fr_slot = nullptr; a.state = nullptr;
  a.partials = nullptr; a.planes = nullptr; a.level = qa.level; a.max_kf = qa.max_kf; a.max_fr = qa.max_fr; a.nblk = qa.nblk; a.save_w = 0;
  FcaAcc acc;
  fca_acc_zero(acc);
  float sc[4] = {0.0f, 0.0f, 0.0f, 0.0f};
  int n_depth = 0, n_used = 0;
  if (c.begin < c.end) {
    const TapRows tr = tap_rows(cur, sw);
    const FcafConst fc = fcaf_const(g, S);
    const int lane = t & 63;
    uint32_t* const q = qbuf[t >> 6];
    int qn = 0;
    uint32_t bxy = 0u;
    int bn = 0;
    DensePix bpx;
    bpx.Z = 1.0f; bpx.var = 0.0f; bpx.I = 0u;
    auto pop = [&](int n) {
      __builtin_amdgcn_wave_barrier();
      bxy = q[qn - n + min(lane, n - 1)];
      __builtin_amdgcn_wave_barrier();
      qn -= n;
      bn = n;
      const unsigned x = bxy & 0xffffu, y = bxy >> 16;
      bpx = dense_request(K, __umul24(y, (unsigned)cols) + x, __umul24(y, (unsigned)sw) + x);
    };
    auto run = [&]() {
      const uint32_t xy = bxy;
      const DensePix px = bpx;
      const bool live = lane < bn;
      bn = 0;
      const int x = (int)(xy & 0xffffu), y = (int)(xy >> 16);
      const unsigned i = __umul24((unsigned)y, (unsigned)cols) + (unsigned)x;
      FcaPix o;
      bool oob;
      if constexpr (FAST) {
        bool valid;
        const FcaInF rec = dense_form(g, px, x, y, valid);
        const FcafStage st = fcaf_stage_a(g, tr, fc, rec);
        o = fcaf_stage_b<false, -1>(a, K, g, cur, fc, i, st);
        oob = tap_oob(cols, g.rows, st.x1, st.y1);
      } else {
// ... 137 lines not shown
```

egomotion_with_local_loop_closures_amd/csrc/ellc_kernels_image.hpp:

```cpp
#pragma once
#include "ellc_device.hpp"

namespace ellc {

#ifndef ELLC_GLOBAL
#define ELLC_GLOBAL __attribute__((address_space(1)))
#endif
template <class T>
__device__ __forceinline__ const ELLC_GLOBAL T* gptr(const T* p) { return (const ELLC_GLOBAL T*)p; }
template <class T>
__device__ __forceinline__ ELLC_GLOBAL T* gptr_rw(T* p) { return (ELLC_GLOBAL T*)p; }

__device__ __forceinline__ int reflect101(int p, int len) {
  if (len == 1) return 0;
  while (p < 0 || p >= len) p = (p < 0) ? -p : 2 * (len - 1) - p;
  return p;
}

__device__ __forceinline__ void grad_at(const uint8_t* __restrict__ img, int sw, int cols, int rows, int x, int y, float& gx, float& gy) {
  const int xm = x > 0 ? x - 1 : 0, xp = x < cols - 1 ? x + 1 : cols - 1;
  const int ym = y > 0 ? y - 1 : 0, yp = y < rows - 1 ? y + 1 : rows - 1;
  const float sx = (x == 0 || x == cols - 1) ? 1.0f : 0.5f;
  const float sy = (y == 0 || y == rows - 1) ? 1.0f : 0.5f;
  const float dx = (float)img[(size_t)y * sw + xp] - (float)img[(size_t)y * sw + xm];
  const float dy = (float)img[(size_t)yp * sw + x] - (float)img[(size_t)ym * sw + x];
  gx = (x == 0 || x == cols - 1) ? dx : 0.5f * dx;
  gy = (y == 0 || y == rows - 1) ? dy : 0.5f * dy;
  (void)sx; (void)sy;
}

__global__ void gradient_planes(const uint8_t* __restrict__ img, int sw, int cols, int rows, float* __restrict__ gx, float* __restrict__ gy) {
  const int x = blockIdx.x * blockDim.x + threadIdx.x;
  const int y = blockIdx.y * blockDim.y + threadIdx.y;
  if (x >= cols || y >= rows) return;
  float a, b;
  grad_at(img, sw, cols, rows, x, y, a, b);
  gx[(size_t)y * cols + x] = a;
  gy[(size_t)y * cols + x] = b;
}

#define ELLC_PT 4
struct PyrChainArgs {
  const uint8_t* src;
  uint8_t* dst[3];
  int w[4], h[4];
  int steps;
};
__device__ __forceinline__ int pyr5(const uint8_t* t, int stride, int x0, int y0, int lox, int loy, int sw, int sh, int x, int y) {
  const int wk[5] = {1, 4, 6, 4, 1};
  int cx[5];
#pragma unroll
  for (int k = 0; k < 5; k++) cx[k] = reflect101(2 * x + k - 2, sw) - lox;
  int v = 0;
#pragma unroll
  for (int j = 0; j < 5; j++) {
    const uint8_t* r = t + (reflect101(2 * y + j - 2, sh) - loy) * stride;
    int hsum = 0;
#pragma unroll
    for (int k = 0; k < 5; k++) hsum += wk[k] * (int)r[cx[k]];
    v += wk[j] * hsum;
  }
  (void)x0; (void)y0;
  return (v + 128) >> 8;
}
__global__ __launch_bounds__(256) void pyr_down_chain_u8(PyrChainArgs a) {
  constexpr int R1 = 2 * ELLC_PT + 3, R2 = 2 * R1 + 3, R3 = 2 * R2 + 3;
  __shared__ uint8_t lds[R3 * R3 + R2 * R2 + R1 * R1];
  const int S = a.steps;
  int lox[4], loy[4], hix[4], hiy[4];
  lox[S] = blockIdx.x * ELLC_PT; loy[S] = blockIdx.y * ELLC_PT;
  hix[S] = min(a.w[S], lox[S] + ELLC_PT); hiy[S] = min(a.h[S], loy[S] + ELLC_PT);
// ... 160 lines not shown
```

include/ellc_abi_diag.h:

```cpp
#ifndef ELLC_ABI_DIAG_H
#define ELLC_ABI_DIAG_H
#include "ellc_abi.h"
#ifdef __cplusplus
extern "C" {
#endif

ellc_status ellc_profile_gn_kernel(ellc_ctx* ctx, int B, const int* kf_slots, const int* frame_slots, int level, int reps,
                                   float* avg_ms, double* algorithmic_bytes, long long* valid_pixels);
ellc_status ellc_profile_align(ellc_ctx* ctx, int B, const int* kf_slots, const int* frame_slots, const float* init_pose,
                               int mode, int reps, float* avg_ms);

ellc_status ellc_profile_depth_stage(ellc_ctx* ctx, int stage, int frame_slot, const float* pose_frame_wrt_kf, int reps, float* avg_ms);

ellc_status ellc_profile_calibrate_read(ellc_ctx* ctx, size_t bytes, int reps, float* avg_ms);
ellc_status ellc_profile_stream_read(ellc_ctx* ctx, size_t bytes, int reps, float* avg_ms);

ellc_status ellc_selftest_div_pair(ellc_ctx* ctx, int n, const float* a, const float* b, float* q_pair, float* q_ref);

ellc_status ellc_selftest_lu(ellc_ctx* ctx, int n, const double* tri21, float* inv36);


ellc_status ellc_debug_schedule_sums(ellc_ctx* ctx, int B, const int* kf_slots, const int* frame_slots, int level, int mode,
                                     const float* pose, double* sums27, float* new_pose, float* ica_hinv36, char* kernel, int kernel_len,
                                     int* grid);

ellc_status ellc_debug_persist_delay(ellc_ctx* ctx, int first_block, int polls);
ellc_status ellc_debug_set_persist_epoch(ellc_ctx* ctx, unsigned epoch);
ellc_status ellc_debug_set_eager_lists(ellc_ctx* ctx, int on);
ellc_status ellc_debug_set_fold_staging(ellc_ctx* ctx, int on);
ellc_status ellc_debug_set_hinv_cache(ellc_ctx* ctx, int on);
ellc_status ellc_debug_set_count_cache(ellc_ctx* ctx, int on);
ellc_status ellc_debug_count_cache_counters(ellc_ctx* ctx, long long* groups_counted, long long* groups_skipped);
ellc_status ellc_debug_persist_counters(ellc_ctx* ctx, long long* resident_launches, long long* abandoned_launches, long long* rejoined_blocks);

#ifdef __cplusplus
}
#endif
#endif
```

Before: 8.927 million GN iterations/s.

## Add column-packed frame planes so fast-mode bilinear taps use one aligned load

Adds a per-frame packed image plane where each 32-bit word holds a pixel and its three vertical neighbours, built by a new pack_tap_rows kernel after pyramid construction. In fast mode the GN tap paths read the 2x2 bilinear neighbourhood with one aligned 8-byte load instead of two unaligned 4-byte row loads. The old row-load path stays available behind a diag-only switch. This costs one packing kernel per frame upload and a fourfold larger extra image buffer per frame level.

New measurement: 9.290 million GN iterations/s (median of 6 runs). 4.1% higher.

```diff
diff --git a/egomotion_with_local_loop_closures_amd/_lib.py b/egomotion_with_local_loop_closures_amd/_lib.py
--- a/egomotion_with_local_loop_closures_amd/_lib.py
+++ b/egomotion_with_local_loop_closures_amd/_lib.py
@@ -26,7 +26,7 @@
 DIAG_SYMBOLS = [
     "ellc_profile_gn_kernel", "ellc_profile_align", "ellc_profile_depth_stage", "ellc_profile_calibrate_read", "ellc_profile_stream_read",
     "ellc_selftest_div_pair", "ellc_selftest_lu", "ellc_debug_persist_delay", "ellc_debug_set_persist_epoch", "ellc_debug_persist_counters", "ellc_debug_set_eager_lists", "ellc_debug_set_hinv_cache", "ellc_debug_set_fold_staging",
-    "ellc_debug_set_count_cache", "ellc_debug_count_cache_counters",
+    "ellc_debug_set_count_cache", "ellc_debug_count_cache_counters", "ellc_debug_set_packed_taps", "ellc_debug_row_tap_launches", "ellc_debug_get_packed_level",
     "ellc_debug_schedule_sums",
 ]
 
diff --git a/egomotion_with_local_loop_closures_amd/api.py b/egomotion_with_local_loop_closures_amd/api.py
--- a/egomotion_with_local_loop_closures_amd/api.py
+++ b/egomotion_with_local_loop_closures_amd/api.py
@@ -327,6 +327,24 @@
     def debug_set_count_cache(self, on):
         self._need_diag("ellc_debug_set_count_cache")
         self._ck(self._l.ellc_debug_set_count_cache(self.h, int(bool(on))), "ellc_debug_set_count_cache")
+
+    def debug_set_packed_taps(self, on):
+        self._need_diag("ellc_debug_set_packed_taps")
+        self._ck(self._l.ellc_debug_set_packed_taps(self.h, int(bool(on))), "ellc_debug_set_packed_taps")
+
+    def debug_row_tap_launches(self):
+        self._need_diag("ellc_debug_row_tap_launches")
+        n = C.c_longlong(0)
+        self._ck(self._l.ellc_debug_row_tap_launches(self.h, C.byref(n)), "ellc_debug_row_tap_launches")
+        return n.value
+
+    def debug_get_packed_level(self, frame_slot, level):
+        self._need_diag("ellc_debug_get_packed_level")
+        sw = C.c_int(0); sh = C.c_int(0)
+        self._ck(self._l.ellc_get_image_level(self.h, 0, int(frame_slot), int(level), None, C.byref(sw), C.byref(sh), None, None), "ellc_get_image_level")
+        out = np.empty((sh.value, sw.value), np.uint32)
+        self._ck(self._l.ellc_debug_get_packed_level(self.h, int(frame_slot), int(level), out.ctypes.data_as(C.c_void_p)), "ellc_debug_get_packed_level")
+        return out
 
     def debug_count_cache_counters(self):
         self._need_diag("ellc_debug_count_cache_counters")
diff --git a/egomotion_with_local_loop_closures_amd/csrc/ellc_context.hpp b/egomotion_with_local_loop_closures_amd/csrc/ellc_context.hpp
--- a/egomotion_with_local_loop_closures_amd/csrc/ellc_context.hpp
+++ b/egomotion_with_local_loop_closures_amd/csrc/ellc_context.hpp
@@ -40,6 +40,7 @@
   bool track = false;
   const void* count_valid = nullptr;
   int count_n = 0;
+  bool row_taps = false;
 };
 
 struct TrackRequest {
@@ -48,16 +49,16 @@
 };
 
 struct GraphKey {
-  int B, nu, mode, save_weights, continuation, track, pollable, adaptive_first, grid_batch, dense, need, skip_count, set;
+  int B, nu, mode, save_weights, continuation, track, pollable, adaptive_first, grid_batch, dense, need, skip_count, set, row_taps;
   bool operator<(const GraphKey& o) const {
     auto t = [](const GraphKey& k) {
-      return std::tie(k.B, k.nu, k.mode, k.save_weights, k.continuation, k.track, k.pollable, k.adaptive_first, k.grid_batch, k.dense, k.need, k.skip_count, k.set);
+      return std::tie(k.B, k.nu, k.mode, k.save_weights, k.continuation, k.track, k.pollable, k.adaptive_first, k.grid_batch, k.dense, k.need, k.skip_count, k.set, k.row_taps);
     };
     return t(*this) < t(o);
   }
 };
 inline GraphKey graph_key(const LaunchPlan& p, int grid_batch) {
-  return GraphKey{p.B, p.nu, p.mode, p.save_weights ? 1 : 0, p.continuation, p.track, p.pollable, p.adaptive_first, grid_batch, p.dense, p.need, p.skip_count, p.set};
+  return GraphKey{p.B, p.nu, p.mode, p.save_weights ? 1 : 0, p.continuation, p.track, p.pollable, p.adaptive_first, grid_batch, p.dense, p.need, p.skip_count, p.set, p.row_taps};
 }
 
 }
@@ -73,6 +74,8 @@
   char* arena_base = nullptr;
   size_t arena_size = 0, arena_used = 0;
   bool fast = false;
+  bool row_taps = false;
+  long long row_tap_args = 0;
   std::vector<void*> host_allocs;
   std::vector<ellc::KfLevelDev> kf_tab_h;
   std::vector<ellc::FrLevelDev> fr_tab_h;
@@ -257,5 +260,6 @@
 ellc_status build_depth_pyramid_from(ellc_ctx* c, int slot, int first_level);
 ellc_status build_maxgrad(ellc_ctx* c, bool is_kf, int slot);
 ellc_status build_image_pyramid(ellc_ctx* c, uint8_t* const* img, hipStream_t st);
+ellc_status pack_frame_taps(ellc_ctx* c, int slot, hipStream_t st);
 ellc_status mark_frame_use(ellc_ctx* c, int slot);
 }
diff --git a/egomotion_with_local_loop_closures_amd/csrc/ellc_device.hpp b/egomotion_with_local_loop_closures_amd/csrc/ellc_device.hpp
--- a/egomotion_with_local_loop_closures_amd/csrc/ellc_device.hpp
+++ b/egomotion_with_local_loop_closures_amd/csrc/ellc_device.hpp
@@ -61,6 +61,7 @@
 
 struct FrLevelDev {
   uint8_t* img;
+  uint32_t* img4;
 };
 
 #define DM_OBS_REGIONS 64
diff --git a/egomotion_with_local_loop_closures_amd/csrc/ellc_hip.hip b/egomotion_with_local_loop_closures_amd/csrc/ellc_hip.hip
--- a/egomotion_with_local_loop_closures_amd/csrc/ellc_hip.hip
+++ b/egomotion_with_local_loop_closures_amd/csrc/ellc_hip.hip
@@ -144,7 +144,25 @@
   return ELLC_OK;
 }
 
-static ellc_status upload_pyramid(ellc_ctx* c, uint8_t* const* img, const uint8_t* host, int frame_slot = -1) {
+ellc_status pack_frame_taps(ellc_ctx* c, int slot, hipStream_t st) {
+  if (!c->fast) return ELLC_OK;
+  PackRowsArgs a;
+  a.levels = c->L;
+  a.begin[0] = 0;
+  for (int l = 0; l < ELLC_MAX_LEVELS; l++) {
+    const int q = std::min(l, c->L - 1);
+    const FrLevelDev& f = c->fr_tab_h[(size_t)q * c->cfg.max_frames + slot];
+    const LevelGeom& g = c->geom_h[q];
+    a.img[l] = f.img; a.img4[l] = f.img4;
+    a.sw[l] = g.sw; a.rows[l] = g.rows;
+    a.begin[l + 1] = a.begin[l] + (l < c->L ? ((g.sw + 3) / 4) * g.sh : 0);
+  }
+  hipLaunchKernelGGL(pack_tap_rows, dim3((a.begin[c->L] + 255) / 256), dim3(256), 0, st, a);
+  ELLC_HIP(c, hipGetLastError());
+  return ELLC_OK;
+}
+
+static ellc_status upload_pyramid(ellc_ctx* c, uint8_t* const* img, const uint8_t* host, int frame_slot = -1, int pack_slot = -1) {
   const LevelGeom* g = c->geom_h;
   hipStream_t st = c->stream;
   if (frame_slot >= 0) {
@@ -180,7 +198,8 @@
     const int blocks = (int)std::min<size_t>(1024, ((bytes >> 4) + 255) / 256 + 1);
     hipLaunchKernelGGL(ingest_copy_u8, dim3(blocks), dim3(256), 0, st, img[0], (const uint8_t*)stage_dev, bytes);
   }
-  const ellc_status s = build_image_pyramid(c, img, st);
+  ellc_status s = build_image_pyramid(c, img, st);
+  if (s == ELLC_OK && pack_slot >= 0) s = pack_frame_taps(c, pack_slot, st);
   ELLC_HIP(c, hipEventRecord(c->upload_done[k], st));
   if (s != ELLC_OK || frame_slot < 0) return s;
   if (!c->fr_ready_ev[frame_slot]) ELLC_HIP(c, hipEventCreateWithFlags(&c->fr_ready_ev[frame_slot], hipEventDisableTiming));
@@ -295,6 +314,10 @@
   a.max_fr = c->cfg.max_frames;
   a.nblk = choose_nblk(c, level, grid_batch(c, p.B), p.dense);
   a.save_w = save_w;
+#ifdef ELLC_ROW_TAPS
+  a.row_taps = p.row_taps ? 1 : 0;
+  if (p.row_taps) c->row_tap_args++;
+#endif
   return a;
 }
 
@@ -865,7 +888,12 @@
       if (!c->fast) TRY(dev_alloc(c, &k.invz, n));
       TRY(dev_alloc(c, &k.irec, n)); TRY(dev_alloc(c, &k.hpart, (size_t)(tiles + 1) * ELLC_PART_STRIDE)); TRY(dev_alloc(c, &k.hinv, 36));
     }
-    for (int s = 0; s < MF; s++) TRY(dev_alloc(c, &c->fr_tab_h[(size_t)l * MF + s].img, ni + (size_t)g.sw + 32));
+    for (int s = 0; s < MF; s++) {
+      FrLevelDev& f = c->fr_tab_h[(size_t)l * MF + s];
+      TRY(dev_alloc(c, &f.img, ni + (size_t)g.sw + 32));
+      f.img4 = nullptr;
+      if (c->fast) TRY(dev_alloc(c, &f.img4, ni + (size_t)g.sw + 32));
+    }
   }
   TRY(dev_alloc(c, &c->kf_tab_d, c->kf_tab_h.size()));
   TRY(dev_alloc(c, &c->fr_tab_d, c->fr_tab_h.size()));
@@ -1114,6 +1142,31 @@
   c->count_cache = on != 0;
   return ELLC_OK;
 }
+ellc_status ellc_debug_set_packed_taps(ellc_ctx* c, int on) {
+  if (!c) return ELLC_ERR_BAD_ARG;
+  ELLC_ENTER(c);
+#ifndef ELLC_ROW_TAPS
+  if (!on) return fail(c, ELLC_ERR_BAD_ARG, "ellc_debug_set_packed_taps: this build was compiled without the row loads (ELLC_NO_ROW_TAPS)");
+#endif
+  c->row_taps = !on;
+  return ELLC_OK;
+}
+ellc_status ellc_debug_row_tap_launches(ellc_ctx* c, long long* n) {
+  if (!c || !n) return ELLC_ERR_BAD_ARG;
+  ELLC_ENTER(c);
+  *n = c->row_tap_args;
+  return ELLC_OK;
+}
+ellc_status ellc_debug_get_packed_level(ellc_ctx* c, int frame_slot, int level, uint32_t* out) {
+  if (!c || !out || level < 0 || level >= c->L || !slot_ok(frame_slot, c->cfg.max_frames)) return fail(c, ELLC_ERR_BAD_ARG, "bad argument");
+  ELLC_ENTER(c);
+  if (!c->fast) return fail(c, ELLC_ERR_NOT_READY, "ellc_debug_get_packed_level: contexts of the exact mode keep no packed planes");
+  if (!c->fr_has_image[frame_slot]) return fail(c, ELLC_ERR_NOT_READY, "slot empty");
+  const LevelGeom& g = c->geom_h[level];
+  ELLC_HIP(c, hipMemcpyAsync(out, c->fr_tab_h[(size_t)level * c->cfg.max_frames + frame_slot].img4, (size_t)g.sw * g.sh * 4, hipMemcpyDeviceToHost, c->stream));
+  ELLC_HIP(c, hipStreamSynchronize(c->stream));
+  return ELLC_OK;
+}
 ellc_status ellc_debug_count_cache_counters(ellc_ctx* c, long long* groups_counted, long long* groups_skipped) {
   if (!c) return ELLC_ERR_BAD_ARG;
   ELLC_ENTER(c);
@@ -1164,7 +1217,7 @@
   uint8_t* img[ELLC_MAX_LEVELS];
   for (int l = 0; l < c->L; l++) img[l] = c->fr_tab_h[(size_t)l * c->cfg.max_frames + slot].img;
   const bool own_stream = c->cfg.concurrent_batches <= 1 && c->coalesce <= 1;
-  ellc_status s = upload_pyramid(c, img, image, own_stream ? slot : -1);
+  ellc_status s = upload_pyramid(c, img, image, own_stream ? slot : -1, slot);
   if (s != ELLC_OK) return s;
   c->fr_has_image[slot] = 1;
   c->fr_maxgrad_valid[slot] = 0;
@@ -1418,6 +1471,7 @@
   } else {
     dc->fr_has_image[dst] = 1;
     dc->fr_maxgrad_valid[dst] = 0;
+    return pack_frame_taps(dc, dst, dc->stream);
   }
   return ELLC_OK;
 }
@@ -1488,6 +1542,7 @@
   p.resident = resident;
   p.adaptive_first = schedule_is_adaptive(c, mode, B) ? adaptive_first_launches(c, resident) : 0;
   p.direct = launches_directly(c, mode, B);
+  p.row_taps = c->row_taps;
   return p;
 }
 
@@ -1885,6 +1940,7 @@
   ellc_status s = stage_batch(c, 1, &kf_slot, &frame_slot, pose, &nu);
   if (s != ELLC_OK) return s;
   LaunchPlan plan;
+  plan.row_taps = c->row_taps;
   plan.B = 1;
   plan.nu = nu;
   plan.mode = mode;
@@ -1986,6 +2042,10 @@
   qa.max_fr = c->cfg.max_frames;
   qa.nblk = quality_nblk(c, level);
   qa.max_batch = MB;
+#ifdef ELLC_ROW_TAPS
+  qa.row_taps = c->row_taps ? 1 : 0;
+  if (c->row_taps) c->row_tap_args++;
+#endif
   const dim3 grd(qa.nblk, B), blk(ELLC_GN_THREADS);
   if (c->fast) hipLaunchKernelGGL((gn_fca_quality<true, false>), grd, blk, 0, c->stream, qa);
   else if (c->geom_h[0].divc_ok) hipLaunchKernelGGL((gn_fca_quality<false, true>), grd, blk, 0, c->stream, qa);
@@ -2007,6 +2067,7 @@
   ellc_status s = stage_batch(c, 1, &kf_slot, &frame_slot, pose, &nu);
   if (s != ELLC_OK) return s;
   LaunchPlan plan;
+  plan.row_taps = c->row_taps;
   plan.B = 1;
   enqueue_stage_in(c, plan, 0);
   hipLaunchKernelGGL(gn_set_pose0, dim3(1), dim3(1), 0, c->stream, c->state_d, c->init_pose_d);
@@ -2065,6 +2126,7 @@
   if (s != ELLC_OK) return s;
   const bool dense = group_is_dense(c, ELLC_MODE_FCA, B, 0, kf_slots, B);
   LaunchPlan plan;
+  plan.row_taps = c->row_taps;
   plan.B = B;
   plan.nu = dense ? 0 : nu;
   plan.dense = dense;
diff --git a/egomotion_with_local_loop_closures_amd/csrc/ellc_ingest_impl.hpp b/egomotion_with_local_loop_closures_amd/csrc/ellc_ingest_impl.hpp
--- a/egomotion_with_local_loop_closures_amd/csrc/ellc_ingest_impl.hpp
+++ b/egomotion_with_local_loop_closures_amd/csrc/ellc_ingest_impl.hpp
@@ -191,6 +191,7 @@
                      g[0].sw, gd, ud);
   hipError_t e = hipGetLastError();
   if (e == hipSuccess && build_image_pyramid(c, img, c->stream) != ELLC_OK) e = hipErrorUnknown;
+  if (e == hipSuccess && pack_frame_taps(c, slot, c->stream) != ELLC_OK) e = hipErrorUnknown;
   if (e == hipSuccess && gd) e = hipMemcpyAsync(gray_probe, gd, (size_t)ow * oh, hipMemcpyDeviceToHost, c->stream);
   if (e == hipSuccess && ud) e = hipMemcpyAsync(undistorted_probe, ud, (size_t)ow * oh * 4, hipMemcpyDeviceToHost, c->stream);
   if (e == hipSuccess) e = hipStreamSynchronize(c->stream);
diff --git a/egomotion_with_local_loop_closures_amd/csrc/ellc_kernels_gn.hpp b/egomotion_with_local_loop_closures_amd/csrc/ellc_kernels_gn.hpp
--- a/egomotion_with_local_loop_closures_amd/csrc/ellc_kernels_gn.hpp
+++ b/egomotion_with_local_loop_closures_amd/csrc/ellc_kernels_gn.hpp
@@ -91,6 +91,14 @@
 __device__ __forceinline__ uint32_t load_u32_unaligned(g_u8 base, unsigned byte_off) {
   return *(const ELLC_GLOBAL u32_align1*)(base + byte_off);
 }
+typedef uint32_t u32x2_t __attribute__((ext_vector_type(2)));
+typedef uint32_t u32x4_t __attribute__((ext_vector_type(4)));
+typedef u32x2_t u32x2_a1 __attribute__((aligned(1)));
+typedef u32x2_t u32x2_a4 __attribute__((aligned(4)));
+typedef u32x4_t u32x4_a4 __attribute__((aligned(4)));
+#if defined(ELLC_DIAG_ABI) && !defined(ELLC_NO_ROW_TAPS)
+#define ELLC_ROW_TAPS 1
+#endif
 template <int N>
 __device__ __forceinline__ float byte_f32(uint32_t w) { return (float)((w >> (8 * N)) & 0xffu); }
 
@@ -211,8 +219,10 @@
 template <class T> struct is_lat_pf { static constexpr bool value = false; };
 template <class F> struct is_lat_pf<LatPF<F>> { static constexpr bool value = true; };
 template <class F> __device__ __forceinline__ LatPF<F> lat_pf(F f) { return LatPF<F>{f}; }
-template <bool WANT_GRAD, bool FAST = false, class AfterIssue = NoPrefetch>
-__device__ __forceinline__ Taps tap_point(g_u8 img, int sw, int cols, int rows, float x1, float y1, AfterIssue after_issue = AfterIssue()) {
+template <bool WANT_GRAD, bool FAST = false, class AfterIssue = NoPrefetch, bool PACKED = false>
+__device__ __forceinline__ Taps tap_point(g_u8 img, int sw, int cols, int rows, float x1, float y1, AfterIssue after_issue = AfterIssue(),
+                                          g_u8 img4 = nullptr, bool row_taps = false) {
+  static_assert(!PACKED || (FAST && !WANT_GRAD), "the packed form serves the tolerance mode's intensity-only taps");
   Taps o;
   const float fx0 = floorf(x1), fy0 = floorf(y1);
   const float wx = x1 - fx0, wy = y1 - fy0;
@@ -222,13 +232,19 @@
     const int x0 = (int)fx0, y0 = (int)fy0;
     uint32_t wa = 0, wb, wc, wd = 0;
     const unsigned ob = __umul24((unsigned)y0, (unsigned)sw) + (unsigned)x0 - 1u, oc = ob + (unsigned)sw;
-    wb = load_u32_unaligned(img, ob);
-    wc = load_u32_unaligned(img, oc);
-    if (WANT_GRAD) { wa = load_u32_unaligned(img, ob - (unsigned)sw); wd = load_u32_unaligned(img, oc + (unsigned)sw); }
+    const bool packed = PACKED && !row_taps;
+    if (packed) {
+      const u32x2_t v = *(const ELLC_GLOBAL u32x2_a4*)(img4 + ((ob + 1u) << 2));
+      wb = v.x; wc = v.y;
+    } else {
+      wb = load_u32_unaligned(img, ob);
+      wc = load_u32_unaligned(img, oc);
+      if (WANT_GRAD) { wa = load_u32_unaligned(img, ob - (unsigned)sw); wd = load_u32_unaligned(img, oc + (unsigned)sw); }
+    }
     __builtin_amdgcn_sched_barrier(0);
     after_issue();
     __builtin_amdgcn_sched_barrier(0);
-    const float Pbb = byte_f32<1>(wb), Pbc = byte_f32<2>(wb), Pcb = byte_f32<1>(wc), Pcc = byte_f32<2>(wc);
+    const float Pbb = byte_f32<1>(wb), Pbc = packed ? byte_f32<1>(wc) : byte_f32<2>(wb), Pcb = packed ? byte_f32<2>(wb) : byte_f32<1>(wc), Pcc = byte_f32<2>(wc);
     if (FAST) {
       const float top = __builtin_fmaf(wx, Pbc - Pbb, Pbb);
       const float btm = __builtin_fmaf(wx, Pcc - Pcb, Pcb);
@@ -274,13 +290,34 @@
   return tap_general<WANT_GRAD, FAST, is_lat_pf<AfterIssue>::value>(img, sw, cols, rows, x1, y1);
 }
 
-struct TapRows { g_u8 ra, rb, rc, rd; };
-__device__ __forceinline__ TapRows tap_rows(g_u8 img, int sw) {
-  TapRows r;
+struct TapRows {
+  g_u8 p4;
+#ifdef ELLC_ROW_TAPS
+  g_u8 ra, rb, rc, rd;
+  bool rows;
+#endif
+};
+struct RowPtrs { g_u8 ra, rb, rc, rd; };
+__device__ __forceinline__ RowPtrs row_ptrs(g_u8 img, int sw) {
+  RowPtrs r;
   r.rb = img - 1;
   r.ra = r.rb - sw;
   r.rc = r.rb + sw;
   r.rd = r.rc + sw;
+  return r;
+}
+struct GnArgs;
+__device__ __forceinline__ bool row_taps_of(const GnArgs& a);
+__device__ __forceinline__ TapRows tap_rows(const GnArgs& a, g_u8 img, g_u8 img4, int sw) {
+  TapRows r;
+  r.p4 = img4 - 4;
+#ifdef ELLC_ROW_TAPS
+  r.rb = img - 1;
+  r.ra = r.rb - sw;
+  r.rc = r.rb + sw;
+  r.rd = r.rc + sw;
+  r.rows = row_taps_of(a);
+#endif
   return r;
 }
 template <int N>
@@ -300,6 +337,9 @@
 struct TapReq {
   uint32_t wa, wb, wc, wd;
   bool interior;
+#ifdef ELLC_ROW_TAPS
+  bool rows;
+#endif
 };
 template <bool WANT_GRAD, class AfterIssue = NoPrefetch>
 __device__ __forceinline__ TapReq tap_request_f(const TapRows& tr, int sw, int cols, int rows, float x1, float y1, AfterIssue after_issue = AfterIssue()) {
@@ -309,6 +349,9 @@
   const bool interior = ((unsigned)(x0 - 1) <= (unsigned)(cols - 4)) & ((unsigned)(y0 - 1) <= (unsigned)(rows - 4));
   q.interior = (__builtin_amdgcn_ballot_w64(!interior) == 0ull);
   q.wb = 0; q.wc = 0;
+#ifdef ELLC_ROW_TAPS
+  q.rows = tr.rows;
+#endif
   if (q.interior) {
     const unsigned off = __umul24((unsigned)y0, (unsigned)sw) + (unsigned)x0;
 #ifdef ELLC_X_LDSTAPS
@@ -318,9 +361,17 @@
     q.wc = __builtin_amdgcn_alignbit(xl[1024 + o + 1], xl[1024 + o], shb);
     if (WANT_GRAD) { q.wa = __builtin_amdgcn_alignbit(xl[2048 + o + 1], xl[2048 + o], shb); q.wd = __builtin_amdgcn_alignbit(xl[3072 + o + 1], xl[3072 + o], shb); }
 #else
-    q.wb = load_u32_unaligned(tr.rb, off);
-    q.wc = load_u32_unaligned(tr.rc, off);
-    if (WANT_GRAD) { q.wa = load_u32_unaligned(tr.ra, off); q.wd = load_u32_unaligned(tr.rd, off); }
+#ifdef ELLC_ROW_TAPS
+    if (tr.rows) {
+      q.wb = load_u32_unaligned(tr.rb, off);
+      q.wc = load_u32_unaligned(tr.rc, off);
+      if (WANT_GRAD) { q.wa = load_u32_unaligned(tr.ra, off); q.wd = load_u32_unaligned(tr.rd, off); }
+    } else
+#endif
+    {
+      const u32x4_t v = *(const ELLC_GLOBAL u32x4_a4*)(tr.p4 + (off << 2));
+      q.wa = v.x; q.wb = v.y; q.wc = v.z; q.wd = v.w;
+    }
 #endif
     __builtin_amdgcn_sched_barrier(0);
     after_issue();
@@ -335,13 +386,22 @@
   if (q.interior) {
     Taps o;
     const float wx = __builtin_amdgcn_fractf(x1), wy = __builtin_amdgcn_fractf(y1);
-    const float Pbb = cvt_ubyte<1>(q.wb), Pbc = cvt_ubyte<2>(q.wb), Pcb = cvt_ubyte<1>(q.wc), Pcc = cvt_ubyte<2>(q.wc);
+    float Pbb = cvt_ubyte<1>(q.wb), Pbc = cvt_ubyte<1>(q.wc), Pcb = cvt_ubyte<2>(q.wb), Pcc = cvt_ubyte<2>(q.wc);
+#ifdef ELLC_ROW_TAPS
+    if (q.rows) { Pbb = cvt_ubyte<1>(q.wb); Pbc = cvt_ubyte<2>(q.wb); Pcb = cvt_ubyte<1>(q.wc); Pcc = cvt_ubyte<2>(q.wc); }
+#endif
     const float top = __builtin_fmaf(wx, Pbc - Pbb, Pbb);
     const float btm = __builtin_fmaf(wx, Pcc - Pcb, Pcb);
     o.I = __builtin_fmaf(wy, btm - top, top);
     if (WANT_GRAD) {
-      const float Pba = cvt_ubyte<0>(q.wb), Pbd = cvt_ubyte<3>(q.wb), Pca = cvt_ubyte<0>(q.wc), Pcd = cvt_ubyte<3>(q.wc);
-      const float Pab = cvt_ubyte<1>(q.wa), Pac = cvt_ubyte<2>(q.wa), Pdb = cvt_ubyte<1>(q.wd), Pdc = cvt_ubyte<2>(q.wd);
+      float Pba = cvt_ubyte<1>(q.wa), Pbd = cvt_ubyte<1>(q.wd), Pca = cvt_ubyte<2>(q.wa), Pcd = cvt_ubyte<2>(q.wd);
+      float Pab = cvt_ubyte<0>(q.wb), Pac = cvt_ubyte<0>(q.wc), Pdb = cvt_ubyte<3>(q.wb), Pdc = cvt_ubyte<3>(q.wc);
+#ifdef ELLC_ROW_TAPS
+      if (q.rows) {
+        Pba = cvt_ubyte<0>(q.wb); Pbd = cvt_ubyte<3>(q.wb); Pca = cvt_ubyte<0>(q.wc); Pcd = cvt_ubyte<3>(q.wc);
+        Pab = cvt_ubyte<1>(q.wa); Pac = cvt_ubyte<2>(q.wa); Pdb = cvt_ubyte<1>(q.wd); Pdc = cvt_ubyte<2>(q.wd);
+      }
+#endif
       const float g00 = Pbc - Pba, g01 = Pbd - Pbb, g10 = Pcc - Pca, g11 = Pcd - Pcb;
       float t2 = __builtin_fmaf(wx, g01 - g00, g00);
       float b2 = __builtin_fmaf(wx, g11 - g10, g10);
@@ -454,7 +514,17 @@
   float* planes;
   int level, max_kf, max_fr, nblk;
   int save_w;
+#ifdef ELLC_ROW_TAPS
+  int row_taps;
+#endif
 };
+__device__ __forceinline__ bool row_taps_of(const GnArgs& a) {
+#ifdef ELLC_ROW_TAPS
+  return a.row_taps != 0;
+#else
+  return false;
+#endif
+}
 
 template <int NV>
 struct WaveRows {
@@ -619,7 +689,6 @@
   return fca_pixel_in<DEBUG, DIVC>(a, K, g, cur, S, i, fca_load<DIVC>(K, g, i));
 }
 
-typedef uint32_t u32x4_t __attribute__((ext_vector_type(4)));
 struct FcaInF { u32x4_t v; };
 __device__ __forceinline__ FcaInF fcaf_empty() { FcaInF in; in.v = (u32x4_t){0u, 0u, 0x3f800000u, 0u}; return in; }
 
@@ -793,9 +862,10 @@
 #pragma unroll
   for (int i = 0; i < 12; i++) S[i] = st.S[i];
   g_u8 cur = as_global(F.img);
+  g_u8 cur4 = (g_u8)as_global(F.img4);
   FcaAcc acc;
   fca_acc_zero(acc);
-  const TapRows tr = tap_rows(cur, g.sw);
+  const TapRows tr = tap_rows(a, cur, cur4, g.sw);
   const FcafConst fc = fcaf_const(g, S);
   for (int i = begin + (int)threadIdx.x; i < end; i += ELLC_GN_THREADS) {
     FcaPix p;
@@ -1488,7 +1558,7 @@
 }
 
 template <bool DIVC, bool PIPE, bool FAST, int SAVEW, bool LAT = false>
-__device__ __forceinline__ void fca_chunk_pass(const GnArgs& a, const KfLevelDev& K, const LevelGeom& g, g_u8 cur, const float* newS, int begin,
+__device__ __forceinline__ void fca_chunk_pass(const GnArgs& a, const KfLevelDev& K, const LevelGeom& g, g_u8 cur, g_u8 cur4, const float* newS, int begin,
                                                int end, const FcaIn& first, const FcaInF& firstf, const FcaPre& first_pre, float (&sums)[27]) {
   constexpr int stride = ELLC_GN_THREADS;
   const int t = threadIdx.x;
@@ -1500,7 +1570,7 @@
   int i = begin + t;
   if constexpr (FAST) {
     if (begin < end) {
-      const TapRows tr = tap_rows(cur, g.sw);
+      const TapRows tr = tap_rows(a, cur, cur4, g.sw);
       const FcafConst fc = fcaf_const(g, S);
       ELLC_PTRACE(4, 0);
       unsigned off = (unsigned)i * ELLC_FREC, idx = (unsigned)i;
@@ -1575,6 +1645,7 @@
   const double group_sum = partial_group_sum(pending_partials(prev_part, b), prev_nblk);
   const Chunk c = m.chunk(fa.age_cum, V, nblk);
   g_u8 cur = as_global(F.img);
+  g_u8 cur4 = (g_u8)as_global(F.img4);
   FirstRec first = no_record();
   request_first<DIVC, FAST, true>(first, K, g, c, t, true);
   advance_pose<FAST>(sh, pending, group_sum, 0, fa.prev_level, fa.early_exit, src);
@@ -1582,7 +1653,7 @@
   ELLC_BSTAMP(1);
   if (publish_level_bound(sh, src, next_state(fa, b), sub == 0, pending, fa.prev_level, a.level)) return;
   float sums[27];
-  fca_chunk_pass<DIVC, PIPE, FAST, SAVEW>(a, K, g, cur, sh.newS, c.begin, c.end, first.in, first.inf, first.pre, sums);
+  fca_chunk_pass<DIVC, PIPE, FAST, SAVEW>(a, K, g, cur, cur4, sh.newS, c.begin, c.end, first.in, first.inf, first.pre, sums);
   ELLC_STAMP(7);
   ELLC_BSTAMP(2);
   block_reduce_store<27>(sums, partial_record(fa, fa.seq, b, sub));
@@ -1632,6 +1703,7 @@
   const double group_sum = partial_group_sum(pending_partials(prev_part, b), prev_nblk);
   const Chunk c = m.chunk(fa.age_cum, g.n, nblk);
   g_u8 cur = as_global(F.img);
+  g_u8 cur4 = (g_u8)as_global(F.img4);
   const int sw = g.sw;
   const PlaneWalk w = plane_walk(g.cols);
   const PlanePos p0 = plane_first(w, c, t);
@@ -1648,7 +1720,7 @@
     FcaAcc acc;
     fca_acc_zero(acc);
     if (c.begin < c.end) {
-      const TapRows tr = tap_rows(cur, sw);
+      const TapRows tr = tap_rows(a, cur, cur4, sw);
       const FcafConst fc = fcaf_const(g, S);
       dense_plane_pass(c, w, sw, p0, pix, [&](unsigned i, unsigned img_off) { return dense_request(K, i, img_off); },
                        [&](const DensePix& px, const PlanePos& p, bool active, auto refill) {
@@ -1725,8 +1797,6 @@
 }
 
 typedef float f32x4_t __attribute__((ext_vector_type(4)));
-typedef uint32_t u32x2_t __attribute__((ext_vector_type(2)));
-typedef u32x2_t u32x2_a1 __attribute__((aligned(1)));
 struct QuadPlanes { f32x4_t Z, var; uint32_t I; };
 __device__ __forceinline__ QuadPlanes quad_request(const KfLevelDev& K, unsigned i4, unsigned img_off) {
   QuadPlanes p;
@@ -1762,6 +1832,7 @@
   const Chunk c = m.chunk(fa.age_cum, g.n >> 2, nblk);
   const int begin = c.begin, end = c.end;
   g_u8 cur = as_global(F.img);
+  g_u8 cur4 = (g_u8)as_global(F.img4);
   const PlaneWalk w = plane_walk(cols4);
   PlanePos p = plane_first(w, c, t);
   QuadPlanes pl;
@@ -1779,8 +1850,9 @@
     FcaAcc acc;
     fca_acc_zero(acc);
     if (begin < end) {
-      const TapRows tr = tap_rows(cur, sw);
-      const g_u8 row_e = tr.rd + sw;
+      const TapRows tr = tap_rows(a, cur, cur4, sw);
+      const RowPtrs rw = row_ptrs(cur, sw);
+      const g_u8 row_e = rw.rd + sw;
       float P[12];
       {
         const FcafConst f0 = fcaf_const(g, S);
@@ -1836,10 +1908,10 @@
                            ((unsigned)(ys - 1) <= (unsigned)(g.rows - 4)) & ((unsigned)(ym - 1) <= (unsigned)(g.rows - 4)) &
                            (xm - xs <= 4) & (ym - ys <= 1);
           const unsigned off = fit ? __umul24((unsigned)ys, (unsigned)sw) + (unsigned)xs : (unsigned)sw + 1u;
-          const u32x2_t wA = *(const ELLC_GLOBAL u32x2_a1*)(tr.ra + off);
-          const u32x2_t wB = *(const ELLC_GLOBAL u32x2_a1*)(tr.rb + off);
-          const u32x2_t wC = *(const ELLC_GLOBAL u32x2_a1*)(tr.rc + off);
-          const u32x2_t wD = *(const ELLC_GLOBAL u32x2_a1*)(tr.rd + off);
+          const u32x2_t wA = *(const ELLC_GLOBAL u32x2_a1*)(rw.ra + off);
+          const u32x2_t wB = *(const ELLC_GLOBAL u32x2_a1*)(rw.rb + off);
+          const u32x2_t wC = *(const ELLC_GLOBAL u32x2_a1*)(rw.rc + off);
+          const u32x2_t wD = *(const ELLC_GLOBAL u32x2_a1*)(rw.rd + off);
           const u32x2_t wE = *(const ELLC_GLOBAL u32x2_a1*)(row_e + off);
           __builtin_amdgcn_sched_barrier(0);
           pl = quad_request(K, inext, __umul24((unsigned)n.y, (unsigned)sw) + 4u * (unsigned)n.x);
@@ -1993,8 +2065,9 @@
     return;
   }
   g_u8 cur = as_global(L.F->img);
+  g_u8 cur4 = (g_u8)as_global(L.F->img4);
   float sums[27];
-  fca_chunk_pass<DIVC, true, FAST, SAVEW>(a, L.K, L.g, cur, sh.newS, L.c.begin, L.c.end, first.in, first.inf, first.pre, sums);
+  fca_chunk_pass<DIVC, true, FAST, SAVEW>(a, L.K, L.g, cur, cur4, sh.newS, L.c.begin, L.c.end, first.in, first.inf, first.pre, sums);
   block_reduce_store<27>(sums, partial_record(fa, fa.seq, b, sub));
 }
 
@@ -2264,8 +2337,9 @@
     }
     if (work) {
       g_u8 cur = as_global(L.F->img);
+      g_u8 cur4 = (g_u8)as_global(L.F->img4);
       float sums[27];
-      fca_chunk_pass<DIVC, true, FAST, SAVEW, true>(a, L.K, L.g, cur, sh.newS, L.c.begin, L.c.end, first.in, first.inf, first.pre, sums);
+      fca_chunk_pass<DIVC, true, FAST, SAVEW, true>(a, L.K, L.g, cur, cur4, sh.newS, L.c.begin, L.c.end, first.in, first.inf, first.pre, sums);
       ELLC_PTRACE(7, 0);
       unsigned* out = (unsigned*)partial_record(fa, seq, b, sub);
       persist_store_record(sums, out, (epoch << 8) | (unsigned)(seq + 1));
@@ -2323,7 +2397,7 @@
 
 template <bool FAST>
 __device__ __forceinline__ void ica_accumulate_pixel(float (&acc)[6], const typename IcaInOf<FAST>::type& in, const LevelGeom& g, g_u8 cur,
-                                                     const float* S) {
+                                                     const float* S, g_u8 cur4 = nullptr, bool row_taps = false) {
   if constexpr (FAST) {
     const float p = __builtin_fmaf((float)(in.xyI & 0xfffu), g.rfx, -(g.cx * g.rfx));
     const float q = __builtin_fmaf((float)((in.xyI >> 12) & 0xfffu), g.rfy, -(g.cy * g.rfy));
@@ -2334,7 +2408,7 @@
     const float rz = __builtin_amdgcn_rcpf(pz);
     const float wx = __builtin_fmaf(px * rz, g.fx, g.cx);
     const float wy = __builtin_fmaf(py * rz, g.fy, g.cy);
-    const Taps t = tap_point<false, true>(cur, g.sw, g.cols, g.rows, wx, wy);
+    const Taps t = tap_point<false, true, NoPrefetch, true>(cur, g.sw, g.cols, g.rows, wx, wy, NoPrefetch(), cur4, row_taps);
     const bool oob = (t.I == -1.0f);
     const float residual = oob ? 0.0f : (t.I - byte_f32<3>(in.xyI));
     const float rw = residual * in.W;
@@ -2375,6 +2449,7 @@
   const Chunk c = m.chunk(fa.age_cum, V, a.nblk);
   const int begin = c.begin, end = c.end;
   g_u8 cur = as_global(F.img);
+  g_u8 cur4 = (g_u8)as_global(F.img4);
   typename IcaInOf<FAST>::type first = ica_in_empty<FAST>();
   if (begin + t < end) first = ica_load_any<FAST>(K, (unsigned)(begin + t));
   advance_pose<FAST>(sh, pending, group_sum, 2, fa.prev_level, fa.early_exit, src, &a.kf_tab[fa.prev_level * a.max_kf + slot].hinv);
@@ -2387,8 +2462,8 @@
   for (int i = 0; i < 6; i++) acc[i] = 0.0f;
   int i = begin + t;
   if (i < end) {
-    ica_accumulate_pixel<FAST>(acc, first, g, cur, S);
-    for (i += ELLC_GN_THREADS; i < end; i += ELLC_GN_THREADS) ica_accumulate_pixel<FAST>(acc, ica_load_any<FAST>(K, (unsigned)i), g, cur, S);
+    ica_accumulate_pixel<FAST>(acc, first, g, cur, S, cur4, row_taps_of(a));
+    for (i += ELLC_GN_THREADS; i < end; i += ELLC_GN_THREADS) ica_accumulate_pixel<FAST>(acc, ica_load_any<FAST>(K, (unsigned)i), g, cur, S, cur4, row_taps_of(a));
   }
   block_reduce_store<6>(acc, partial_record(fa, fa.seq, b, sub) + 21);
 }
@@ -2630,6 +2705,9 @@
   int* counts;
   QualityRec* out;
   int level, max_kf, max_fr, nblk, max_batch;
+#ifdef ELLC_ROW_TAPS
+  int row_taps;
+#endif
 };
 
 __device__ __forceinline__ bool tap_oob(int cols, int rows, float x1, float y1) {
@@ -2651,6 +2729,7 @@
   const KfLevelDev K = qa.kf_tab[qa.level * qa.max_kf + qa.stage[b]];
   const FrLevelDev& F = qa.fr_tab[qa.level * qa.max_fr + qa.stage[qa.max_batch + b]];
   g_u8 cur = as_global(F.img);
+  g_u8 cur4 = (g_u8)as_global(F.img4);
   Chunk c;
   {
     const int n = (g.n + qa.nblk - 1) / qa.nblk;
@@ -2683,12 +2762,15 @@
   GnArgs a;
   a.geom = qa.geom; a.kf_tab = qa.kf_tab; a.fr_tab = qa.fr_tab; a.kf_slot = nullptr; a.fr_slot = nullptr; a.state = nullptr;
   a.partials = nullptr; a.planes = nullptr; a.level = qa.level; a.max_kf = qa.max_kf; a.max_fr = qa.max_fr; a.nblk = qa.nblk; a.save_w = 0;
+#ifdef ELLC_ROW_TAPS
+  a.row_taps = qa.row_taps;
+#endif
   FcaAcc acc;
   fca_acc_zero(acc);
   float sc[4] = {0.0f, 0.0f, 0.0f, 0.0f};
   int n_depth = 0, n_used = 0;
   if (c.begin < c.end) {
-    const TapRows tr = tap_rows(cur, sw);
+    const TapRows tr = tap_rows(a, cur, cur4, sw);
     const FcafConst fc = fcaf_const(g, S);
     const int lane = t & 63;
     uint32_t* const q = qbuf[t >> 6];
diff --git a/egomotion_with_local_loop_closures_amd/csrc/ellc_kernels_image.hpp b/egomotion_with_local_loop_closures_amd/csrc/ellc_kernels_image.hpp
--- a/egomotion_with_local_loop_closures_amd/csrc/ellc_kernels_image.hpp
+++ b/egomotion_with_local_loop_closures_amd/csrc/ellc_kernels_image.hpp
@@ -37,6 +37,37 @@
   grad_at(img, sw, cols, rows, x, y, a, b);
   gx[(size_t)y * cols + x] = a;
   gy[(size_t)y * cols + x] = b;
+}
+
+struct PackRowsArgs {
+  const uint8_t* img[ELLC_MAX_LEVELS];
+  uint32_t* img4[ELLC_MAX_LEVELS];
+  int sw[ELLC_MAX_LEVELS], rows[ELLC_MAX_LEVELS];
+  int begin[ELLC_MAX_LEVELS + 1];
+  int levels;
+};
+__global__ __launch_bounds__(256) void pack_tap_rows(PackRowsArgs a) {
+  typedef uint32_t u32_a1 __attribute__((aligned(1)));
+  const int t = blockIdx.x * 256 + threadIdx.x;
+  if (t >= a.begin[a.levels]) return;
+  int l = 0;
+#pragma unroll
+  for (int k = 1; k < ELLC_MAX_LEVELS; k++) if (k < a.levels && t >= a.begin[k]) l = k;
+  const int sw = a.sw[l], rows = a.rows[l], q = (sw + 3) >> 2;
+  const int i = t - a.begin[l], y = i / q, x = (i - y * q) * 4;
+  const ELLC_GLOBAL uint8_t* img = gptr(a.img[l]);
+  uint32_t r[4];
+#pragma unroll
+  for (int k = 0; k < 4; k++) {
+    const int yy = y - 1 + k;
+    r[k] = (yy >= 0 && yy < rows) ? *(const ELLC_GLOBAL u32_a1*)(img + (size_t)yy * sw + x) : 0u;
+  }
+  ELLC_GLOBAL uint32_t* out = gptr_rw(a.img4[l]) + (size_t)y * sw + x;
+#pragma unroll
+  for (int k = 0; k < 4; k++) {
+    const uint32_t w = ((r[0] >> (8 * k)) & 0xffu) | (((r[1] >> (8 * k)) & 0xffu) << 8) | (((r[2] >> (8 * k)) & 0xffu) << 16) | (((r[3] >> (8 * k)) & 0xffu) << 24);
+    if (x + k < sw) out[k] = w;
+  }
 }
 
 #define ELLC_PT 4
diff --git a/include/ellc_abi_diag.h b/include/ellc_abi_diag.h
--- a/include/ellc_abi_diag.h
+++ b/include/ellc_abi_diag.h
@@ -31,6 +31,9 @@
 ellc_status ellc_debug_set_hinv_cache(ellc_ctx* ctx, int on);
 ellc_status ellc_debug_set_count_cache(ellc_ctx* ctx, int on);
 ellc_status ellc_debug_count_cache_counters(ellc_ctx* ctx, long long* groups_counted, long long* groups_skipped);
+ellc_status ellc_debug_set_packed_taps(ellc_ctx* ctx, int on);
+ellc_status ellc_debug_row_tap_launches(ellc_ctx* ctx, long long* n);
+ellc_status ellc_debug_get_packed_level(ellc_ctx* ctx, int frame_slot, int level, uint32_t* out);
 ellc_status ellc_debug_persist_counters(ellc_ctx* ctx, long long* resident_launches, long long* abandoned_launches, long long* rejoined_blocks);
 
 #ifdef __cplusplus
```
